# okieraised/rs-face-detection

Hardware: AMD Instinct MI355X
Metric: images/sec + p50 latency, RetinaFace-R50 640x640 b32 (end-to-end detect: preprocess + CNN + decode + NMS; `value` = frames resident in HBM, `value_host_path` = SURVEY 8(d)'s H2D -> ... -> D2H figure) (higher is better)
Workload: dtype bf16; 1 GPU; RetinaFace-ResNet50 640x640 batch=32 bf16 per GPU (BASELINE.json configs[2]); batch_per_gpu=32, global_batch=32, max_det=1024, parallelism=single GPU

## Files before the change

### include/rfd.h

```cpp
#ifndef RFD_H
#define RFD_H

#include <stddef.h>
#include <stdint.h>

#ifdef __cplusplus
extern "C" {
#endif

#define RFD_VERSION 1

#if defined(__GNUC__)
#define RFD_API __attribute__((visibility("default")))
#else
#define RFD_API
#endif

typedef enum rfd_status {
    RFD_OK = 0,
    RFD_ERR_INVALID_ARG = -1,
    RFD_ERR_NO_DEVICE = -2,
    RFD_ERR_HIP = -3,
    RFD_ERR_CAPACITY = -4,
    RFD_ERR_STATE = -5,
// ... 144 lines not shown
    float minimum_face_ratio;
} rfd_selection_config;
RFD_API void rfd_selection_config_default(rfd_selection_config *cfg);
RFD_API int rfd_select_faces(rfd_ctx *ctx, const rfd_dets *dets, const int *img_h, const int *img_w, int n,
                             const rfd_selection_config *cfg, int is_enroll, float *out_box, float *out_kps,
                             int32_t *found);
RFD_API int rfd_detect_select_batch(rfd_ctx *ctx, const rfd_image *imgs, int n, const rfd_selection_config *cfg,
                                    int is_enroll, float *out_box, float *out_kps, int32_t *found);

RFD_API int rfd_host_alloc(size_t bytes, void **ptr);
RFD_API int rfd_host_free(void *ptr);
RFD_API int rfd_submit_batch(rfd_ctx *ctx, const rfd_image *imgs, int n);
RFD_API int rfd_collect_batch(rfd_ctx *ctx, rfd_dets *out, int *n_out);

typedef struct rfd_alignment_config {
    int32_t out_w, out_h;
    float standard_landmarks[10];
    int32_t reserved[4];
} rfd_alignment_config;
RFD_API void rfd_alignment_config_default(rfd_alignment_config *cfg);
RFD_API int rfd_align_faces(rfd_ctx *ctx, const rfd_image *imgs, int n, const float *boxes, const float *kps,
                            const int32_t *found, const rfd_alignment_config *cfg, uint8_t *out_crops,
                            int32_t *status);
RFD_API int rfd_detect_select_align_batch(rfd_ctx *ctx, const rfd_image *imgs, int n,
                                          const rfd_selection_config *sel_cfg, int is_enroll,
                                          const rfd_alignment_config *align_cfg, float *out_box, float *out_kps,
                                          int32_t *found, uint8_t *out_crops, int32_t *status);

#define RFD_MAX_FACE_TENSORS 4
typedef struct rfd_face_tensor_config {
    int32_t out_w, out_h;
    float   mean[3];
    float   scale[3];
    int32_t reserved[4];
} rfd_face_tensor_config;
RFD_API void rfd_face_tensor_config_quality(rfd_face_tensor_config *cfg);
RFD_API void rfd_face_tensor_config_extraction(rfd_face_tensor_config *cfg);
RFD_API int rfd_face_tensors(rfd_ctx *ctx, const uint8_t *crops, int n, int crop_w, int crop_h,
                             const rfd_face_tensor_config *cfgs, int k, float *const *tensors);
RFD_API int rfd_detect_select_align_tensors_batch(rfd_ctx *ctx, const rfd_image *imgs, int n,
                                                  const rfd_selection_config *sel_cfg, int is_enroll,
                                                  const rfd_alignment_config *align_cfg, float *out_box, float *out_kps,
                                                  int32_t *found, uint8_t *out_crops, int32_t *status,
                                                  const rfd_face_tensor_config *cfgs, int k, float *const *tensors);
RFD_API int rfd_align_faces_tensors(rfd_ctx *ctx, const rfd_image *imgs, int n, const float *boxes, const float *kps,
                                    const int32_t *found, const rfd_alignment_config *cfg, uint8_t *out_crops,
                                    int32_t *status, const rfd_face_tensor_config *cfgs, int k, float *const *tensors);
typedef struct rfd_faces {
    float *box;
    float *kps;
    int32_t *found;
    uint8_t *crops;
    int32_t *status;
    float *tensors[RFD_MAX_FACE_TENSORS];
} rfd_faces;
RFD_API int rfd_detect_faces_device(rfd_ctx *ctx, const rfd_image *imgs, int n, const rfd_selection_config *sel_cfg,
                                    int is_enroll, const rfd_alignment_config *align_cfg,
                                    const rfd_face_tensor_config *cfgs, int k, rfd_faces *out, int async);
RFD_API int rfd_quality_decide(rfd_ctx *ctx, const float *logits, int n, int classes, float threshold, float *score,
                               int32_t *klass);
RFD_API int rfd_normalize_embeddings(rfd_ctx *ctx, const float *emb, int n, int dim, float *out);
RFD_API int rfd_quality_decide_device(rfd_ctx *ctx, const float *logits, int n, int classes, float threshold, float *score,
                                      int32_t *klass);
RFD_API int rfd_normalize_embeddings_device(rfd_ctx *ctx, const float *emb, int n, int dim, float *out);

RFD_API int rfd_get_stats(rfd_ctx *ctx, rfd_stats *stats);
RFD_API int rfd_get_config(const rfd_ctx *ctx, rfd_config *cfg);
RFD_API int rfd_set_thresholds(rfd_ctx *ctx, float confidence_threshold, float iou_threshold);
RFD_API int rfd_set_profiling(rfd_ctx *ctx, int enable);
RFD_API int rfd_get_conv_profile(rfd_ctx *ctx, float *ms_conv, double *flops_conv, int *launches);
RFD_API int rfd_get_op_profile(rfd_ctx *ctx, float *ms, int cap);

RFD_API int rfd_debug_tensor_io(rfd_ctx *ctx, int tensor_id, int n, void *host, int write);
RFD_API int rfd_debug_run_ops(rfd_ctx *ctx, int n, int first_op, int last_op);
RFD_API int rfd_debug_run_chain(rfd_ctx *ctx, int n, int first_op, int last_op, int batch_off, int co_running);
RFD_API int rfd_debug_pass_chains(rfd_ctx *ctx, int n, int *sizes, int cap);
RFD_API int rfd_debug_buffer_io(rfd_ctx *ctx, int tensor_id, void *host, size_t bytes, int write, size_t *image_pitch);
RFD_API int rfd_debug_set_conv_tile(rfd_ctx *ctx, int tile);
RFD_API int rfd_debug_op_kernels(rfd_ctx *ctx, int n, int op, int co_running, char *names, int cap);
RFD_API int rfd_debug_op_kernels_static(int backbone, int net_w, int net_h, int n, int op, int co_running, int tile, int schedule,
                                        int cus, char *names, int cap);
RFD_API int rfd_debug_set_concurrency(rfd_ctx *ctx, int multi_stream, int split_min_part, int split_max_parts,
                                      int use_graph);

RFD_API int rfd_debug_poke_nms_flag(rfd_ctx *ctx, int value);
RFD_API int rfd_debug_persistent_kernel(int i, const char **name, size_t *lds_bytes);

#ifdef __cplusplus
}
#endif
#endif
```

### rs-face-detection_amd/csrc/detector.hip

```cpp
#include <dlfcn.h>
#include <stdarg.h>
#include <stdlib.h>

#include <mutex>
#include <vector>

#include "network.h"

namespace rfd {

static thread_local char g_err[512] = "";

void set_error(const char *fmt, ...)
{
    va_list ap;
    va_start(ap, fmt);
    vsnprintf(g_err, sizeof g_err, fmt, ap);
    va_end(ap);
}
const char *get_error() { return g_err; }

static void make_base_anchors(float out[kNumLevels][kA][4])
{
    static const float scales[kNumLevels][kA] = {{32.f, 16.f}, {8.f, 4.f}, {2.f, 1.f}};
// ... 98 lines not shown
    g_rccl = r;
    return RFD_OK;
}

#define RFD_RCCL(expr)                                                                                      \
    do {                                                                                                    \
        const int _r = (expr);                                                                              \
        if (_r != 0) {                                                                                      \
            ::rfd::set_error("%s failed: %s (%s:%d)", #expr, g_rccl.GetErrorString(_r), __FILE__, __LINE__); \
            return RFD_ERR_COMM;                                                                            \
        }                                                                                                   \
    } while (0)

struct DevBuf {
    void *p = nullptr;
    size_t cap = 0;
    int reserve(size_t bytes)
    {
        if (bytes <= cap) return RFD_OK;
        if (p) RFD_HIP(hipFree(p));
        p = nullptr; cap = 0;
        RFD_HIP(hipMalloc(&p, bytes));
        cap = bytes;
        return RFD_OK;
    }
    void release() { if (p) (void)hipFree(p); p = nullptr; cap = 0; }
};

}

using namespace rfd;

struct rfd_ctx {
    rfd_config cfg;
    hipStream_t stream = nullptr;
    hipStream_t own_stream = nullptr;
    hipEvent_t ev[10] = {};
    float base_anchor[kNumLevels][kA][4];
    int fh[kNumLevels], fw[kNumLevels], level_off[kNumLevels], total_anchors = 0;
    Network net;
    bool net_created = false;
    DevBuf staging, imgs, in4, rows, keys, sorted_keys, sorted_boxes, count, det_scale;
    DevBuf nms_kept, nms_state;
    int nms_epoch = 0;
    int nms_ticket_sel = 0;
    bool nms_chunked = true;
    int *h_nms_flag = nullptr;
    DevBuf out_boxes, out_lmk, out_count, out_total, out_gidx;
    DevBuf scratch[12];
    DevBuf sel_dims, sel_out;
    DevBuf align_faces, align_out, align_status;
    DevBuf face_in, face_tensors[kMaxFaceTensors], face_io[2];
    static constexpr int kRing = 4;
    PreImage *pin_imgs[kRing] = {};
    float *pin_scales[kRing] = {};
    hipEvent_t pin_done[kRing] = {};
    int pin_next = 0;
    int *pin_dims[kRing] = {};
    hipEvent_t pin_dims_done[kRing] = {};
    int pin_dims_next = 0;
    struct PipeSlot {
        DevBuf frames, imgs, scale, ob, ol, oc, ot;
        PreImage *pin_imgs = nullptr;
        float *pin_scale = nullptr;
        float *h_ob = nullptr, *h_ol = nullptr;
        int *h_oc = nullptr, *h_ot = nullptr;
        hipEvent_t h2d = nullptr, done = nullptr, post = nullptr;
        int n = 0;
    };
    static constexpr int kPipe = 2;
    static constexpr int kPipeRows = 128;
    PipeSlot pipe[kPipe];
    hipStream_t copy_stream = nullptr, d2h_stream = nullptr;
    int pipe_head = 0, pipe_tail = 0, pipe_inflight = 0;
    DevBuf ov_imgs[2], ov_scale[2];
    hipEvent_t ov_chain_done[2][2] = {}, ov_post_done[2] = {}, ov_desc = nullptr;
    bool ov_post_valid[2] = {false, false};
    int ov_parity = 0;
    int ov_last_n = -1;
    hipEvent_t ov_resync = nullptr;
    Rccl::Comm comm = nullptr;
    int comm_rank = 0, comm_world = 0;
    rfd_stats stats;
    float conv_ms = 0.f;
    double conv_flops = 0.0;
    int conv_launches = 0;

    int ensure_network()
    {
        if (net_created) return RFD_OK;
        RFD_TRY(net.create(cfg.backbone, cfg.image_w, cfg.image_h, cfg.max_batch_size, cfg.precision, cfg.schedule));
        net.d_fail = (int *)nms_state.p + (size_t)cfg.max_batch_size * kNmsChunks * 2;
        net_created = true;
        return RFD_OK;
    }
};

namespace {

int ctx_alloc(rfd_ctx *c)
{
    const size_t B = (size_t)c->cfg.max_batch_size, NA = (size_t)c->total_anchors, MD = (size_t)c->cfg.max_det;
    RFD_TRY(c->imgs.reserve(B * sizeof(PreImage)));
    RFD_TRY(c->rows.reserve(B * NA * kDetRow * sizeof(float)));
    RFD_TRY(c->keys.reserve(B * NA * sizeof(uint64_t)));
    RFD_TRY(c->sorted_keys.reserve(B * NA * sizeof(uint64_t)));
    RFD_TRY(c->sorted_boxes.reserve(B * NA * sizeof(float4)));
    RFD_TRY(c->nms_kept.reserve(B * NA * sizeof(float4)));
    RFD_TRY(c->nms_state.reserve((B * kNmsChunks * 2 + 4) * sizeof(int)));
    RFD_HIP(hipMemset(c->nms_state.p, 0, (B * kNmsChunks * 2 + 4) * sizeof(int)));
    RFD_HIP(hipDeviceSynchronize());
    RFD_TRY(c->count.reserve(B * sizeof(int)));
    RFD_TRY(c->det_scale.reserve(B * sizeof(float)));
    RFD_TRY(c->out_boxes.reserve(B * MD * 5 * sizeof(float)));
    RFD_TRY(c->out_lmk.reserve(B * MD * 10 * sizeof(float)));
    RFD_TRY(c->out_count.reserve(B * sizeof(int)));
    RFD_TRY(c->out_total.reserve(B * sizeof(int)));
    RFD_TRY(c->out_gidx.reserve(B * MD * sizeof(int)));
    return RFD_OK;
}

int check_images(const rfd_ctx *c, const rfd_image *imgs, int n)
{
    RFD_CHECK_ARG(imgs != nullptr, "imgs is null");
    if (n < 1 || n > c->cfg.max_batch_size) {
        set_error("batch of %d frames exceeds max_batch_size %d", n, c->cfg.max_batch_size);
        return RFD_ERR_CAPACITY;
    }
    for (int i = 0; i < n; ++i) {
        RFD_CHECK_ARG(imgs[i].data != nullptr, "frame data is null");
        RFD_CHECK_ARG(imgs[i].height > 0 && imgs[i].width > 0, "frame has a non-positive size");
        RFD_CHECK_ARG(imgs[i].stride >= (ptrdiff_t)imgs[i].width * 3, "frame stride < width*3 (frames must be 3-channel 8-bit)");
    }
    return RFD_OK;
}

int stage_frames(rfd_ctx *c, const rfd_image *imgs, int n, bool frames_on_device, std::vector<float> &scales)
{
    const int slot = c->pin_next;
    c->pin_next = (c->pin_next + 1) % rfd_ctx::kRing;
    RFD_HIP(hipEventSynchronize(c->pin_done[slot]));
    PreImage *pis = c->pin_imgs[slot];
    scales.resize(n);
    size_t total = 0;
    for (int i = 0; i < n; ++i) total += (size_t)imgs[i].height * imgs[i].width * 3;
    if (!frames_on_device) RFD_TRY(c->staging.reserve(total));
    size_t off = 0;
    for (int i = 0; i < n; ++i) {
        letterbox(imgs[i].height, imgs[i].width, c->cfg.image_w, c->cfg.image_h, &pis[i], &scales[i]);
        if (pis[i].new_w <= 0 || pis[i].new_h <= 0) {
            set_error("invalid argument: frame %d (%dx%d) letterboxes to an empty %dx%d image", i, imgs[i].width,
                      imgs[i].height, pis[i].new_w, pis[i].new_h);
            return RFD_ERR_INVALID_ARG;
        }
        if (frames_on_device) {
            pis[i].src = imgs[i].data;
            pis[i].stride = (long long)imgs[i].stride;
        } else {
            uint8_t *dst = (uint8_t *)c->staging.p + off;
            const size_t row = (size_t)imgs[i].width * 3;
            RFD_HIP(hipMemcpy2DAsync(dst, row, imgs[i].data, (size_t)imgs[i].stride, row, imgs[i].height,
                                     hipMemcpyHostToDevice, c->stream));
            pis[i].src = dst;
            pis[i].stride = (long long)row;
            off += row * imgs[i].height;
        }
    }
    memcpy(c->pin_scales[slot], scales.data(), n * sizeof(float));
    RFD_HIP(hipMemcpyAsync(c->imgs.p, pis, n * sizeof(PreImage), hipMemcpyHostToDevice, c->stream));
    RFD_HIP(hipMemcpyAsync(c->det_scale.p, c->pin_scales[slot], n * sizeof(float), hipMemcpyHostToDevice, c->stream));
    RFD_HIP(hipEventRecord(c->pin_done[slot], c->stream));
    return RFD_OK;
}

void fill_decode_params(const rfd_ctx *c, DecodeParams &p)
{
    memset(&p, 0, sizeof p);
    for (int l = 0; l < kNumLevels; ++l) {
        p.fh[l] = c->fh[l]; p.fw[l] = c->fw[l]; p.stride[l] = kStrides[l]; p.level_off[l] = c->level_off[l];
    }
    memcpy(p.base_anchor, c->base_anchor, sizeof p.base_anchor);
    p.total_anchors = c->total_anchors;
    p.net_h = c->cfg.image_h; p.net_w = c->cfg.image_w;
    p.conf_thr = c->cfg.confidence_threshold;
    p.rows = (float *)c->rows.p;
    p.keys = (uint64_t *)c->keys.p;
    p.count = (int *)c->count.p;
}

int post_network(rfd_ctx *c, DecodeParams &dp, bool nchw, int n, float *oboxes, float *olmk, int *ocount,
                 int *ototal, int *ogidx, const float *det_scale = nullptr)
{
    RFD_HIP(hipMemsetAsync(c->count.p, 0, n * sizeof(int), c->stream));
    RFD_TRY(launch_decode(dp, n, nchw, c->stream));
    RFD_HIP(hipEventRecord(c->ev[4], c->stream));
    RFD_TRY(launch_sort((uint64_t *)c->keys.p, (const int *)c->count.p, (const float *)c->rows.p,
                        (uint64_t *)c->sorted_keys.p, (float4 *)c->sorted_boxes.p, c->total_anchors, n, c->stream));
    RFD_HIP(hipEventRecord(c->ev[5], c->stream));
    NmsParams np;
    memset(&np, 0, sizeof np);
    np.sorted_keys = (const uint64_t *)c->sorted_keys.p;
    np.sorted_boxes = (const float4 *)c->sorted_boxes.p;
    np.rows = (const float *)c->rows.p;
    np.count = (const int *)c->count.p;
    np.det_scale = det_scale ? det_scale : (const float *)c->det_scale.p;
    np.presorted_n = -1;
    np.total_anchors = c->total_anchors;
    np.max_det = c->cfg.max_det;
    np.iou_thr = c->cfg.iou_threshold;
    np.out_boxes = oboxes; np.out_lmk = olmk; np.out_count = ocount; np.out_total = ototal; np.out_gidx = ogidx;
    if (c->nms_chunked) {
        np.kept_boxes = (float4 *)c->nms_kept.p;
        np.chunk_state = (int *)c->nms_state.p;
        np.spin_fail = (int *)c->nms_state.p + (size_t)c->cfg.max_batch_size * kNmsChunks * 2;
        np.ticket = (unsigned *)(np.spin_fail + 2);
        np.ticket_sel = c->nms_ticket_sel;
        c->nms_epoch = c->nms_epoch == 0x7fffffff ? 1 : c->nms_epoch + 1;
        np.epoch = c->nms_epoch;
    }
    bool used_chunked = false;
    RFD_TRY(launch_nms(np, n, c->stream, &used_chunked));
    if (used_chunked) c->nms_ticket_sel ^= 1;
    RFD_HIP(hipEventRecord(c->ev[6], c->stream));
    RFD_HIP(hipMemcpyAsync(c->h_nms_flag, (int *)c->nms_state.p + (size_t)c->cfg.max_batch_size * kNmsChunks * 2, sizeof(int), hipMemcpyDeviceToHost, c->stream));
    return RFD_OK;
}

int check_nms_flag(rfd_ctx *c)
{
    if (!c->h_nms_flag || *c->h_nms_flag == 0) return RFD_OK;
    *c->h_nms_flag = 0;
    int *flag = (int *)c->nms_state.p + (size_t)c->cfg.max_batch_size * kNmsChunks * 2;
    RFD_HIP(hipMemsetAsync(flag, 0, sizeof(int), c->stream));
    RFD_HIP(hipStreamSynchronize(c->stream));
    set_error("a device-side bounded wait gave up (chunked NMS: a workgroup waiting for its predecessor chunk; ring convolution: a "
              "wave waiting for a ring slot; split-K convolution: an arrival counter left dirty by an earlier fault); the detections of the batches since the last synchronisation are invalid "
              "(re-submit them; RFD_NMS_CHUNKED=0 selects the one-workgroup-per-image NMS kernel, RFD_CONV_RING=0 the barrier-per-step convolutions)");
    return RFD_ERR_HIP;
}

int finish_stats(rfd_ctx *c, int n, bool have_pre, bool have_net)
{
    float ms;
    memset(&c->stats, 0, sizeof c->stats);
    auto el = [&](int a, int b) { return hipEventElapsedTime(&ms, c->ev[a], c->ev[b]) == hipSuccess ? ms : 0.f; };
    if (have_pre) { c->stats.ms_h2d = el(0, 1); c->stats.ms_preprocess = el(1, 2); }
    if (have_net) c->stats.ms_network = el(2, 3);
    c->stats.ms_decode = el(3, 4);
    c->stats.ms_sort = el(4, 5);
    c->stats.ms_nms = el(5, 6);
    c->stats.ms_d2h = el(6, 7);
    c->stats.ms_total = el(have_pre ? 0 : (have_net ? 2 : 3), 7);
    std::vector<int> cnt(n), tot(n);
    RFD_HIP(hipMemcpy(cnt.data(), c->count.p, n * sizeof(int), hipMemcpyDeviceToHost));
    for (int i = 0; i < n; ++i) c->stats.candidates += cnt[i];
    if (c->net_created && c->net.profiling) {
        RFD_TRY(c->net.collect_profile());
        c->conv_ms = 0.f; c->conv_flops = 0.0; c->conv_launches = 0;
        for (size_t i = 0; i < c->net.g.ops.size(); ++i)
            if (c->net.g.ops[i].kind == OP_CONV || c->net.g.ops[i].kind == OP_B2B) {
                c->conv_ms += c->net.op_ms[i];
                c->conv_flops += 2.0 * c->net.g.layer_macs((int)i) * n;
                ++c->conv_launches;
            }
    }
    return RFD_OK;
}

int detect_overlapped(rfd_ctx *c, const rfd_image *imgs, int n, rfd_dets *out, hipEvent_t frames_ready = nullptr)
{
    Network &net = c->net;
    RFD_TRY(net.ensure_alt_heads());
    const size_t B = (size_t)c->cfg.max_batch_size;
    if (!c->ov_desc) {
        RFD_HIP(hipEventCreateWithFlags(&c->ov_desc, hipEventDisableTiming));
        RFD_HIP(hipEventCreateWithFlags(&c->ov_resync, hipEventDisableTiming));
        for (int a = 0; a < 2; ++a) {
            RFD_HIP(hipEventCreateWithFlags(&c->ov_post_done[a], hipEventDisableTiming));
            for (int b = 0; b < 2; ++b) RFD_HIP(hipEventCreateWithFlags(&c->ov_chain_done[a][b], hipEventDisableTiming));
            RFD_TRY(c->ov_imgs[a].reserve(B * sizeof(PreImage)));
            RFD_TRY(c->ov_scale[a].reserve(B * sizeof(float)));
        }
    }
    const int par = (c->ov_parity ^= 1);
    const int slot = c->pin_next;
    c->pin_next = (c->pin_next + 1) % rfd_ctx::kRing;
    RFD_HIP(hipEventSynchronize(c->pin_done[slot]));
    PreImage *pis = c->pin_imgs[slot];
    for (int i = 0; i < n; ++i) {
        letterbox(imgs[i].height, imgs[i].width, c->cfg.image_w, c->cfg.image_h, &pis[i], &c->pin_scales[slot][i]);
        if (pis[i].new_w <= 0 || pis[i].new_h <= 0) {
            set_error("invalid argument: frame %d (%dx%d) letterboxes to an empty image", i, imgs[i].width, imgs[i].height);
            return RFD_ERR_INVALID_ARG;
        }
        pis[i].src = imgs[i].data;
        pis[i].stride = (long long)imgs[i].stride;
    }
    hipStream_t st[2] = {net.part_stream[0], net.part_stream[1]};
    if (c->ov_last_n != n) {
        RFD_HIP(hipEventRecord(c->ov_resync, c->stream));
        for (int p = 0; p < 2; ++p) RFD_HIP(hipStreamWaitEvent(st[p], c->ov_resync, 0));
    }
    c->ov_last_n = n;
    if (frames_ready)
        for (int p = 0; p < 2; ++p) RFD_HIP(hipStreamWaitEvent(st[p], frames_ready, 0));
    if (c->ov_post_valid[par])
        for (int p = 0; p < 2; ++p) RFD_HIP(hipStreamWaitEvent(st[p], c->ov_post_done[par], 0));
    RFD_HIP(hipMemcpyAsync(c->ov_imgs[par].p, pis, n * sizeof(PreImage), hipMemcpyHostToDevice, st[0]));
    RFD_HIP(hipMemcpyAsync(c->ov_scale[par].p, c->pin_scales[slot], n * sizeof(float), hipMemcpyHostToDevice, st[0]));
    RFD_HIP(hipEventRecord(c->pin_done[slot], st[0]));
    RFD_HIP(hipEventRecord(c->ov_desc, st[0]));
    RFD_HIP(hipStreamWaitEvent(st[1], c->ov_desc, 0));
    net.head_parity = par;
    net.co_running = 1;
    int chain[Network::kMaxParts];
    if (net.pass_chains(n, chain) != 2) { set_error("overlapped calls run as two chains"); return RFD_ERR_STATE; }
    const int B0 = chain[0];
    const size_t in_px = (size_t)c->cfg.image_h * c->cfg.image_w * 4;
    int status = RFD_OK;
    for (int p = 0; p < 2 && status == RFD_OK; ++p) {
        const int off = p ? B0 : 0, Bp = chain[p];
        PreParams pp;
        memset(&pp, 0, sizeof pp);
        pp.imgs = (const PreImage *)c->ov_imgs[par].p + off;
        pp.net_h = c->cfg.image_h; pp.net_w = c->cfg.image_w;
        pp.out_nhwc4 = (bf16_t *)net.tensor_ptr(net.g.input) + (size_t)off * in_px;
        status = launch_preprocess(pp, Bp, st[p]);
        if (status == RFD_OK) status = net.run(Bp, st[p], 0, -1, off, p);
        if (status == RFD_OK && hipEventRecord(c->ov_chain_done[par][p], st[p]) != hipSuccess) status = RFD_ERR_HIP;
    }
    net.co_running = 0;
    if (status != RFD_OK) { net.head_parity = 0; c->ov_last_n = -1; return status; }
    for (int p = 0; p < 2; ++p) RFD_HIP(hipStreamWaitEvent(c->stream, c->ov_chain_done[par][p], 0));
    DecodeParams dp;
    fill_decode_params(c, dp);
    for (int l = 0; l < kNumLevels; ++l) dp.cls[l] = (const float *)net.tensor_ptr(net.g.heads[l]);
    net.head_parity = 0;
    RFD_TRY(post_network(c, dp, false, n, out->boxes, out->landmarks, out->count, out->total, nullptr,
                         (const float *)c->ov_scale[par].p));
    RFD_HIP(hipEventRecord(c->ov_post_done[par], c->stream));
    c->ov_post_valid[par] = true;
    return RFD_OK;
}

int detect_impl(rfd_ctx *c, const rfd_image *imgs, int n, rfd_dets *out, bool on_device, int async, bool frames_on_device)
{
    RFD_CHECK_ARG(c != nullptr, "ctx is null");
    RFD_CHECK_ARG(out && out->boxes && out->landmarks && out->count, "output buffers are null");
    RFD_TRY(check_images(c, imgs, n));
    RFD_TRY(c->ensure_network());
    if (!c->net.weights_ready) { set_error("network weights are not initialised"); return RFD_ERR_STATE; }
    if (async == 2 && on_device && frames_on_device && !c->net.profiling && c->net.multi_stream && c->net.num_parts(n) == 2) {
        RFD_HIP(hipSetDevice(c->cfg.device_id));
        return detect_overlapped(c, imgs, n, out);
    }
    RFD_HIP(hipSetDevice(c->cfg.device_id));
    c->ov_last_n = -1;
    std::vector<float> scales;
    RFD_HIP(hipEventRecord(c->ev[0], c->stream));
    RFD_TRY(stage_frames(c, imgs, n, frames_on_device, scales));
    RFD_HIP(hipEventRecord(c->ev[1], c->stream));
    PreParams pp;
    memset(&pp, 0, sizeof pp);
    pp.imgs = (const PreImage *)c->imgs.p;
    pp.net_h = c->cfg.image_h; pp.net_w = c->cfg.image_w;
    pp.out_nhwc4 = (bf16_t *)c->net.tensor_ptr(c->net.g.input);
    RFD_TRY(launch_preprocess(pp, n, c->stream));
    RFD_HIP(hipEventRecord(c->ev[2], c->stream));
    RFD_TRY(c->net.run_graphed(n, c->stream));
    RFD_HIP(hipEventRecord(c->ev[3], c->stream));
    DecodeParams dp;
    fill_decode_params(c, dp);
    for (int l = 0; l < kNumLevels; ++l) dp.cls[l] = (const float *)c->net.tensor_ptr(c->net.g.heads[l]);
    float *ob = on_device ? out->boxes : (float *)c->out_boxes.p;
    float *ol = on_device ? out->landmarks : (float *)c->out_lmk.p;
    int *oc = on_device ? out->count : (int *)c->out_count.p;
    int *ot = on_device ? out->total : (int *)c->out_total.p;
    RFD_TRY(post_network(c, dp, false, n, ob, ol, oc, ot, nullptr));
    if (!on_device) {
        const size_t MD = (size_t)c->cfg.max_det;
        RFD_HIP(hipMemcpyAsync(out->boxes, ob, n * MD * 5 * sizeof(float), hipMemcpyDeviceToHost, c->stream));
        RFD_HIP(hipMemcpyAsync(out->landmarks, ol, n * MD * 10 * sizeof(float), hipMemcpyDeviceToHost, c->stream));
        RFD_HIP(hipMemcpyAsync(out->count, oc, n * sizeof(int), hipMemcpyDeviceToHost, c->stream));
        if (out->total) RFD_HIP(hipMemcpyAsync(out->total, ot, n * sizeof(int), hipMemcpyDeviceToHost, c->stream));
    }
    RFD_HIP(hipEventRecord(c->ev[7], c->stream));
    if (async && on_device) return RFD_OK;
    RFD_HIP(hipStreamSynchronize(c->stream));
    RFD_TRY(check_nms_flag(c));
    RFD_TRY(finish_stats(c, n, true, true));
    if (!on_device)
        for (int i = 0; i < n; ++i) c->stats.detections += out->total ? out->total[i] : out->count[i];
    return RFD_OK;
}

std::mutex g_nms_mu;
rfd_ctx *g_nms_ctx[16] = {};

}

extern "C" {

void rfd_config_default(rfd_config *cfg)
{
    if (!cfg) return;
    memset(cfg, 0, sizeof *cfg);
    cfg->image_w = 640;
    cfg->image_h = 640;
    cfg->max_batch_size = 1;
    cfg->confidence_threshold = 0.7f;
    cfg->iou_threshold = 0.45f;
    cfg->device_id = 0;
    cfg->max_det = 1024;
    cfg->max_src_w = 3840;
    cfg->max_src_h = 2160;
    cfg->backbone = RFD_BACKBONE_R50;
}

int rfd_version(void) { return RFD_VERSION; }
const char *rfd_last_error(void) { return get_error(); }

int rfd_create(const rfd_config *cfg, rfd_ctx **out)
{
    RFD_CHECK_ARG(cfg && out, "cfg/out is null");
    *out = nullptr;
    RFD_CHECK_ARG(cfg->image_w > 0 && cfg->image_h > 0 && cfg->image_w % 32 == 0 && cfg->image_h % 32 == 0,
                  "image_size must be positive multiples of 32");
    RFD_CHECK_ARG(cfg->max_batch_size >= 1, "max_batch_size < 1");
    RFD_CHECK_ARG(cfg->max_det >= 1, "max_det < 1");
    RFD_CHECK_ARG(cfg->precision == RFD_PRECISION_BF16 || cfg->precision == RFD_PRECISION_F32, "precision must be RFD_PRECISION_BF16 or RFD_PRECISION_F32");
    RFD_CHECK_ARG(cfg->precision == RFD_PRECISION_BF16 || cfg->backbone == RFD_BACKBONE_R50, "the f32 parity mode exists for RetinaFace-R50 only");
    RFD_CHECK_ARG(cfg->schedule == RFD_SCHEDULE_THROUGHPUT || cfg->schedule == RFD_SCHEDULE_LATENCY, "schedule must be RFD_SCHEDULE_THROUGHPUT or RFD_SCHEDULE_LATENCY");
    RFD_CHECK_ARG(cfg->schedule == RFD_SCHEDULE_THROUGHPUT || cfg->precision == RFD_PRECISION_BF16, "the latency schedule exists for the bf16 path only (not the f32 parity mode)");
    int ndev = 0;
    if (hipGetDeviceCount(&ndev) != hipSuccess || ndev <= 0) {
        set_error("no HIP device is available: librfd_hip has no CPU fallback");
        return RFD_ERR_NO_DEVICE;
    }
    if (cfg->device_id < 0 || cfg->device_id >= ndev) {
        set_error("device_id %d out of range (%d devices)", cfg->device_id, ndev);
        return RFD_ERR_NO_DEVICE;
    }
    if (hipSetDevice(cfg->device_id) != hipSuccess) {
        set_error("hipSetDevice(%d) failed", cfg->device_id);
        return RFD_ERR_NO_DEVICE;
    }
    rfd_ctx *c = new rfd_ctx();
    c->cfg = *cfg;
    if (const char *e = getenv("RFD_NMS_CHUNKED")) c->nms_chunked = atoi(e) != 0;
    make_base_anchors(c->base_anchor);
    int off = 0;
    for (int l = 0; l < kNumLevels; ++l) {
// ... 170 lines not shown
    return RFD_OK;
}
int rfd_graph_op(const rfd_graph *gg, int idx, rfd_op_desc *d)
{
    RFD_CHECK_ARG(gg && d, "null argument");
    const Graph *g = reinterpret_cast<const Graph *>(gg);
    RFD_CHECK_ARG(idx >= 0 && idx < (int)g->ops.size(), "op index out of range");
    const Op &o = g->ops[idx];
    memset(d, 0, sizeof *d);
    d->kind = o.kind; d->layer = o.layer; d->in = o.in; d->out = o.out; d->out2 = o.out2; d->outf = o.outf;
    d->res = o.res; d->relu = o.relu; d->res_up2 = o.res_up2; d->res_post = o.res_post;
    d->head_softmax = o.head_softmax; d->y_coff = o.y_coff;
    d->in2 = o.in2; d->layer2 = o.layer2; d->in_affine = o.in_affine;
    d->layer_n2 = o.layer_n2; d->x_coff = o.x_coff; d->y_split = o.y_split; d->y_split_add = o.y_split_add;
    d->n_valid = o.n_valid; d->layer_b = o.layer_b; d->out_b = o.out_b; d->branch = o.branch;
    d->macs = g->layer_macs(idx);
    return RFD_OK;
}
int rfd_graph_tensor(const rfd_graph *gg, int idx, rfd_tensor_desc *d)
{
    RFD_CHECK_ARG(gg && d, "null argument");
    const Graph *g = reinterpret_cast<const Graph *>(gg);
    RFD_CHECK_ARG(idx >= 0 && idx < (int)g->tensors.size(), "tensor index out of range");
    const TensorDesc &t = g->tensors[idx];
    memset(d, 0, sizeof *d);
    d->channels = t.C; d->channels_logical = t.C_logical; d->height = t.H; d->width = t.W; d->is_f32 = t.is_f32;
    d->buffer = t.buffer;
    d->is_input = idx == g->input;
    for (int l = 0; l < 3; ++l)
        if (g->heads[l] == idx) d->head_level = l + 1;
    return RFD_OK;
}
double rfd_graph_macs(const rfd_graph *gg)
{
    return gg ? reinterpret_cast<const Graph *>(gg)->macs_per_image() : 0.0;
}
double rfd_graph_workspace_bytes(const rfd_graph *gg)
{
    if (!gg) return 0.0;
    double s = 0;
    for (size_t b : reinterpret_cast<const Graph *>(gg)->buffer_bytes_per_image) s += (double)b;
    return s;
}

int rfd_debug_tensor_io(rfd_ctx *c, int tensor_id, int n, void *host, int write)
{
    RFD_CHECK_ARG(c && host, "null argument");
    RFD_HIP(hipSetDevice(c->cfg.device_id));
    RFD_TRY(c->ensure_network());
    RFD_CHECK_ARG(tensor_id >= 0 && tensor_id < (int)c->net.g.tensors.size(), "tensor id out of range");
    RFD_CHECK_ARG(n >= 1 && n <= c->cfg.max_batch_size, "batch out of range");
    const size_t bytes = c->net.g.tensors[tensor_id].bytes_per_image() * (size_t)n;
    c->ov_last_n = -1;
    if (c->net.precision != 0 && !c->net.g.tensors[tensor_id].is_f32 && tensor_id != c->net.g.input) {
        set_error("f32 parity mode: intermediate tensors are f32, not the bf16 layout this hook transfers");
        return RFD_ERR_STATE;
    }
    if (write) RFD_HIP(hipMemcpyAsync(c->net.tensor_ptr(tensor_id), host, bytes, hipMemcpyHostToDevice, c->stream));
    else RFD_HIP(hipMemcpyAsync(host, c->net.tensor_ptr(tensor_id), bytes, hipMemcpyDeviceToHost, c->stream));
    RFD_HIP(hipStreamSynchronize(c->stream));
    return RFD_OK;
}
int rfd_debug_set_conv_tile(rfd_ctx *c, int tile)
{
    RFD_CHECK_ARG(c && tile >= 0 && tile <= 31, "bad argument");
    RFD_TRY(c->ensure_network());
    c->net.force_tile = tile;
    return RFD_OK;
}
int rfd_debug_set_concurrency(rfd_ctx *c, int multi_stream, int split_min_part, int split_max_parts, int use_graph)
{
    RFD_CHECK_ARG(c, "ctx is null");
    RFD_TRY(c->ensure_network());
    RFD_HIP(hipStreamSynchronize(c->stream));
    c->net.multi_stream = multi_stream != 0;
    c->net.split_min_part = split_min_part;
    c->net.split_max_parts = split_max_parts;
    c->net.tuned = false;
    c->net.use_graph = use_graph != 0;
    for (hipGraphExec_t &ge : c->net.graph_exec)
        if (ge) { (void)hipGraphExecDestroy(ge); ge = nullptr; }
    return RFD_OK;
}
int rfd_debug_poke_nms_flag(rfd_ctx *c, int value)
{
    RFD_CHECK_ARG(c, "ctx is null");
    RFD_HIP(hipSetDevice(c->cfg.device_id));
    int *flag = (int *)c->nms_state.p + (size_t)c->cfg.max_batch_size * kNmsChunks * 2;
    RFD_HIP(hipMemcpyAsync(flag, &value, sizeof(int), hipMemcpyHostToDevice, c->stream));
    RFD_HIP(hipStreamSynchronize(c->stream));
    return RFD_OK;
}
int rfd_debug_persistent_kernel(int i, const char **name, size_t *lds_bytes) { return rfd::persistent_kernel_table(i, name, lds_bytes); }
int rfd_debug_run_ops(rfd_ctx *c, int n, int first_op, int last_op)
{
    RFD_CHECK_ARG(c, "ctx is null");
    RFD_HIP(hipSetDevice(c->cfg.device_id));
    RFD_TRY(c->ensure_network());
    c->ov_last_n = -1;
    RFD_TRY(c->net.run(n, c->stream, first_op, last_op));
    RFD_HIP(hipMemcpyAsync(c->h_nms_flag, c->net.d_fail, sizeof(int), hipMemcpyDeviceToHost, c->stream));
    RFD_HIP(hipStreamSynchronize(c->stream));
    if (c->net.profiling) RFD_TRY(c->net.collect_profile());
    return check_nms_flag(c);
}

int rfd_debug_run_chain(rfd_ctx *c, int n, int first_op, int last_op, int batch_off, int co_running)
{
    RFD_CHECK_ARG(c, "ctx is null");
    RFD_HIP(hipSetDevice(c->cfg.device_id));
    RFD_TRY(c->ensure_network());
    RFD_CHECK_ARG(n >= 1 && batch_off >= 0 && batch_off + n <= c->cfg.max_batch_size, "chain [batch_off, batch_off + n) out of range");
    c->ov_last_n = -1;
    const int saved = c->net.co_running;
    c->net.co_running = co_running != 0;
    const int st = c->net.run(n, c->stream, first_op, last_op, batch_off, 0);
    c->net.co_running = saved;
    RFD_TRY(st);
    RFD_HIP(hipMemcpyAsync(c->h_nms_flag, c->net.d_fail, sizeof(int), hipMemcpyDeviceToHost, c->stream));
    RFD_HIP(hipStreamSynchronize(c->stream));
    if (c->net.profiling) RFD_TRY(c->net.collect_profile());
    return check_nms_flag(c);
}
int rfd_debug_pass_chains(rfd_ctx *c, int n, int *sizes, int cap)
{
    RFD_CHECK_ARG(c && sizes, "null argument");
    RFD_TRY(c->ensure_network());
    RFD_CHECK_ARG(n >= 1 && n <= c->cfg.max_batch_size, "batch out of range");
    int chain[Network::kMaxParts];
    const int P = c->net.pass_chains(n, chain);
    RFD_CHECK_ARG(cap >= P, "sizes holds fewer entries than the pass has chains");
    for (int p = 0; p < P; ++p) sizes[p] = chain[p];
    return P;
}
int rfd_debug_buffer_io(rfd_ctx *c, int tensor_id, void *host, size_t bytes, int write, size_t *image_pitch)
{
    RFD_CHECK_ARG(c, "ctx is null");
    RFD_HIP(hipSetDevice(c->cfg.device_id));
    RFD_TRY(c->ensure_network());
    RFD_CHECK_ARG(tensor_id >= 0 && tensor_id < (int)c->net.g.tensors.size(), "tensor id out of range");
    if (c->net.precision != 0) { set_error("f32 parity mode keeps its own workspace"); return RFD_ERR_STATE; }
    const size_t pitch = c->net.g.buffer_bytes_per_image[c->net.g.tensors[tensor_id].buffer];
    if (image_pitch) *image_pitch = pitch;
    if (!host) return RFD_OK;
    RFD_CHECK_ARG(bytes == pitch * (size_t)c->cfg.max_batch_size, "bytes is not the size of the buffer (max_batch_size * image pitch)");
    c->ov_last_n = -1;
    if (write) RFD_HIP(hipMemcpyAsync(c->net.tensor_ptr(tensor_id), host, bytes, hipMemcpyHostToDevice, c->stream));
    else RFD_HIP(hipMemcpyAsync(host, c->net.tensor_ptr(tensor_id), bytes, hipMemcpyDeviceToHost, c->stream));
    RFD_HIP(hipStreamSynchronize(c->stream));
    return RFD_OK;
}

int rfd_debug_op_kernels(rfd_ctx *c, int n, int op, int co_running, char *names, int cap)
{
    RFD_CHECK_ARG(c && names && cap > 0, "null argument");
    RFD_HIP(hipSetDevice(c->cfg.device_id));
    RFD_TRY(c->ensure_network());
    RFD_CHECK_ARG(n >= 1 && n <= c->cfg.max_batch_size && op >= 0 && op < (int)c->net.g.ops.size(), "batch or op out of range");
    if (c->net.precision != 0) { set_error("kernel-choice introspection covers the bf16 path"); return RFD_ERR_STATE; }
    if (!c->net.weights_ready) { set_error("network weights are not initialised (rfd_init_synthetic_weights / rfd_set_layer_weights)"); return RFD_ERR_STATE; }
    const int saved = c->net.co_running;
    c->net.co_running = co_running != 0;
    std::string out;
    const int st = c->net.op_kernel_names(n, op, device_cus(), &out);
    c->net.co_running = saved;
    RFD_TRY(st);
    snprintf(names, (size_t)cap, "%s", out.c_str());
    return RFD_OK;
}

int rfd_debug_op_kernels_static(int backbone, int net_w, int net_h, int n, int op, int co_running, int tile, int schedule, int cus, char *names, int cap)
{
    RFD_CHECK_ARG(names && cap > 0 && n >= 1 && cus >= 1 && tile >= 0 && tile <= 31, "bad argument");
    Network net;
    RFD_TRY(net.g.build(backbone, net_w, net_h));
    RFD_CHECK_ARG(op >= 0 && op < (int)net.g.ops.size(), "op out of range");
    net.max_batch = n;
    net.schedule = schedule;
    net.force_tile = tile;
    net.co_running = co_running != 0;
    if (schedule == RFD_SCHEDULE_LATENCY) (void)net.plan_splitk();
    char *const base = reinterpret_cast<char *>((uintptr_t)1 << 32);
    net.d_w = reinterpret_cast<bf16_t *>(base);
    net.d_b = reinterpret_cast<float *>(base);
    net.d_zero = reinterpret_cast<bf16_t *>(base);
    net.d_buffers.assign(net.g.buffer_bytes_per_image.size(), base);
    for (int b = 0; b < 3; ++b) net.d_sk_ws[b] = reinterpret_cast<float *>(base);
    net.d_sk_cnt = reinterpret_cast<unsigned *>(base);
    std::string out;
    RFD_TRY(net.op_kernel_names(n, op, cus, &out));
    snprintf(names, (size_t)cap, "%s", out.c_str());
    return RFD_OK;
}

int rfd_init_synthetic_weights(rfd_ctx *c, uint64_t seed)
{
    RFD_CHECK_ARG(c, "ctx is null");
    RFD_HIP(hipSetDevice(c->cfg.device_id));
    RFD_TRY(c->ensure_network());
    return c->net.init_synthetic(seed, c->stream);
}
int rfd_num_layers(const rfd_ctx *c)
{
    if (!c || !c->net_created) return 0;
    return (int)c->net.g.layers.size();
// ... 198 lines not shown
}
int rfd_host_free(void *ptr)
{
    if (ptr) RFD_HIP(hipHostFree(ptr));
    return RFD_OK;
}

int rfd_submit_batch(rfd_ctx *c, const rfd_image *imgs, int n)
{
    RFD_CHECK_ARG(c != nullptr, "ctx is null");
    RFD_TRY(check_images(c, imgs, n));
    if (c->pipe_inflight >= rfd_ctx::kPipe) {
        set_error("%d batches are already in flight: call rfd_collect_batch first", c->pipe_inflight);
        return RFD_ERR_STATE;
    }
    RFD_HIP(hipSetDevice(c->cfg.device_id));
    RFD_TRY(c->ensure_network());
    const size_t B = (size_t)c->cfg.max_batch_size, MD = (size_t)c->cfg.max_det;
    rfd_ctx::PipeSlot &ps = c->pipe[c->pipe_head];
    if (!c->copy_stream) RFD_HIP(hipStreamCreateWithFlags(&c->copy_stream, hipStreamNonBlocking));
    if (!ps.done) {
        RFD_HIP(hipEventCreateWithFlags(&ps.h2d, hipEventDisableTiming));
        RFD_HIP(hipEventCreateWithFlags(&ps.done, hipEventDisableTiming));
        RFD_HIP(hipHostMalloc((void **)&ps.pin_imgs, B * sizeof(PreImage), hipHostMallocDefault));
        RFD_HIP(hipHostMalloc((void **)&ps.pin_scale, B * sizeof(float), hipHostMallocDefault));
        RFD_HIP(hipHostMalloc((void **)&ps.h_ob, B * MD * 5 * sizeof(float), hipHostMallocDefault));
        RFD_HIP(hipHostMalloc((void **)&ps.h_ol, B * MD * 10 * sizeof(float), hipHostMallocDefault));
        RFD_HIP(hipHostMalloc((void **)&ps.h_oc, B * sizeof(int), hipHostMallocDefault));
        RFD_HIP(hipHostMalloc((void **)&ps.h_ot, B * sizeof(int), hipHostMallocDefault));
        RFD_TRY(ps.imgs.reserve(B * sizeof(PreImage)));
        RFD_TRY(ps.scale.reserve(B * sizeof(float)));
        RFD_TRY(ps.ob.reserve(B * MD * 5 * sizeof(float)));
        RFD_TRY(ps.ol.reserve(B * MD * 10 * sizeof(float)));
        RFD_TRY(ps.oc.reserve(B * sizeof(int)));
        RFD_TRY(ps.ot.reserve(B * sizeof(int)));
    }
    size_t total = 0;
    for (int i = 0; i < n; ++i) total += (size_t)imgs[i].height * imgs[i].width * 3;
    if (total > ps.frames.cap) {
        RFD_TRY(ps.frames.reserve(total + total / 4));
    }
    size_t off = 0;
    for (int i = 0; i < n; ++i) {
        letterbox(imgs[i].height, imgs[i].width, c->cfg.image_w, c->cfg.image_h, &ps.pin_imgs[i], &ps.pin_scale[i]);
        if (ps.pin_imgs[i].new_w <= 0 || ps.pin_imgs[i].new_h <= 0) {
            set_error("invalid argument: frame %d (%dx%d) letterboxes to an empty image", i, imgs[i].width, imgs[i].height);
            return RFD_ERR_INVALID_ARG;
        }
        ps.pin_imgs[i].src = (uint8_t *)ps.frames.p + off;
        ps.pin_imgs[i].stride = (long long)imgs[i].width * 3;
        off += (size_t)imgs[i].width * 3 * imgs[i].height;
    }
    for (int i = 0; i < n;) {
        size_t bytes = (size_t)imgs[i].width * 3 * imgs[i].height;
        int j = i + 1;
        if (imgs[i].stride == (ptrdiff_t)imgs[i].width * 3) {
            while (j < n && imgs[j].stride == (ptrdiff_t)imgs[j].width * 3 && imgs[j].data == imgs[i].data + bytes) {
                bytes += (size_t)imgs[j].width * 3 * imgs[j].height;
                ++j;
            }
            RFD_HIP(hipMemcpyAsync((void *)ps.pin_imgs[i].src, imgs[i].data, bytes, hipMemcpyHostToDevice, c->copy_stream));
        } else {
            const size_t row = (size_t)imgs[i].width * 3;
            RFD_HIP(hipMemcpy2DAsync((void *)ps.pin_imgs[i].src, row, imgs[i].data, (size_t)imgs[i].stride, row, imgs[i].height,
                                     hipMemcpyHostToDevice, c->copy_stream));
        }
        i = j;
    }
    RFD_HIP(hipMemcpyAsync(ps.imgs.p, ps.pin_imgs, n * sizeof(PreImage), hipMemcpyHostToDevice, c->copy_stream));
    RFD_HIP(hipMemcpyAsync(ps.scale.p, ps.pin_scale, n * sizeof(float), hipMemcpyHostToDevice, c->copy_stream));
    RFD_HIP(hipEventRecord(ps.h2d, c->copy_stream));
    if (!c->net.profiling && c->net.multi_stream && c->net.num_parts(n) == 2 && c->net.weights_ready) {
        std::vector<rfd_image> dev(n);
        for (int i = 0; i < n; ++i) {
            dev[i].data = (const uint8_t *)ps.pin_imgs[i].src; dev[i].height = imgs[i].height; dev[i].width = imgs[i].width;
            dev[i].stride = (ptrdiff_t)imgs[i].width * 3;
        }
        rfd_dets dd;
        dd.boxes = (float *)ps.ob.p; dd.landmarks = (float *)ps.ol.p; dd.count = (int *)ps.oc.p; dd.total = (int *)ps.ot.p;
        RFD_TRY(detect_overlapped(c, dev.data(), n, &dd, ps.h2d));
    } else {
        c->ov_last_n = -1;
        RFD_HIP(hipStreamWaitEvent(c->stream, ps.h2d, 0));
        PreParams pp;
        memset(&pp, 0, sizeof pp);
        pp.imgs = (const PreImage *)ps.imgs.p;
        pp.net_h = c->cfg.image_h; pp.net_w = c->cfg.image_w;
        pp.out_nhwc4 = (bf16_t *)c->net.tensor_ptr(c->net.g.input);
        RFD_TRY(launch_preprocess(pp, n, c->stream));
        RFD_TRY(c->net.run_graphed(n, c->stream));
        DecodeParams dp;
        fill_decode_params(c, dp);
        for (int l = 0; l < kNumLevels; ++l) dp.cls[l] = (const float *)c->net.tensor_ptr(c->net.g.heads[l]);
        RFD_TRY(post_network(c, dp, false, n, (float *)ps.ob.p, (float *)ps.ol.p, (int *)ps.oc.p, (int *)ps.ot.p, nullptr,
                             (const float *)ps.scale.p));
    }
    if (!c->d2h_stream) RFD_HIP(hipStreamCreateWithFlags(&c->d2h_stream, hipStreamNonBlocking));
    if (!ps.post) RFD_HIP(hipEventCreateWithFlags(&ps.post, hipEventDisableTiming));
    RFD_HIP(hipEventRecord(ps.post, c->stream));
    RFD_HIP(hipStreamWaitEvent(c->d2h_stream, ps.post, 0));
    const size_t R = std::min<size_t>(MD, rfd_ctx::kPipeRows);
    RFD_HIP(hipMemcpy2DAsync(ps.h_ob, MD * 5 * sizeof(float), ps.ob.p, MD * 5 * sizeof(float), R * 5 * sizeof(float), n, hipMemcpyDeviceToHost, c->d2h_stream));
    RFD_HIP(hipMemcpy2DAsync(ps.h_ol, MD * 10 * sizeof(float), ps.ol.p, MD * 10 * sizeof(float), R * 10 * sizeof(float), n, hipMemcpyDeviceToHost, c->d2h_stream));
    RFD_HIP(hipMemcpyAsync(ps.h_oc, ps.oc.p, n * sizeof(int), hipMemcpyDeviceToHost, c->d2h_stream));
    RFD_HIP(hipMemcpyAsync(ps.h_ot, ps.ot.p, n * sizeof(int), hipMemcpyDeviceToHost, c->d2h_stream));
    RFD_HIP(hipEventRecord(ps.done, c->d2h_stream));
    ps.n = n;
    c->pipe_head = (c->pipe_head + 1) % rfd_ctx::kPipe;
    ++c->pipe_inflight;
    return RFD_OK;
}

int rfd_collect_batch(rfd_ctx *c, rfd_dets *out, int *n_out)
{
    RFD_CHECK_ARG(c && out && out->boxes && out->landmarks && out->count, "null argument");
    if (c->pipe_inflight <= 0) { set_error("no batch in flight"); return RFD_ERR_STATE; }
    rfd_ctx::PipeSlot &ps = c->pipe[c->pipe_tail];
    RFD_HIP(hipEventSynchronize(ps.done));
    if (*c->h_nms_flag) {
        c->pipe_tail = (c->pipe_tail + 1) % rfd_ctx::kPipe;
        --c->pipe_inflight;
        return check_nms_flag(c);
    }
    const size_t MD = (size_t)c->cfg.max_det;
    bool more = false;
    for (int i = 0; i < ps.n; ++i)
        if ((size_t)ps.h_oc[i] > (size_t)rfd_ctx::kPipeRows) {
            const size_t R = rfd_ctx::kPipeRows, k = (size_t)ps.h_oc[i];
            RFD_HIP(hipMemcpyAsync(ps.h_ob + ((size_t)i * MD + R) * 5, (const float *)ps.ob.p + ((size_t)i * MD + R) * 5, (k - R) * 5 * sizeof(float), hipMemcpyDeviceToHost, c->d2h_stream));
            RFD_HIP(hipMemcpyAsync(ps.h_ol + ((size_t)i * MD + R) * 10, (const float *)ps.ol.p + ((size_t)i * MD + R) * 10, (k - R) * 10 * sizeof(float), hipMemcpyDeviceToHost, c->d2h_stream));
            more = true;
        }
    if (more) RFD_HIP(hipStreamSynchronize(c->d2h_stream));
    for (int i = 0; i < ps.n; ++i) {
        const int k = ps.h_oc[i];
        memcpy(out->boxes + (size_t)i * MD * 5, ps.h_ob + (size_t)i * MD * 5, (size_t)k * 5 * sizeof(float));
        memcpy(out->landmarks + (size_t)i * MD * 10, ps.h_ol + (size_t)i * MD * 10, (size_t)k * 10 * sizeof(float));
        out->count[i] = k;
        if (out->total) out->total[i] = ps.h_ot[i];
    }
    if (n_out) *n_out = ps.n;
    c->pipe_tail = (c->pipe_tail + 1) % rfd_ctx::kPipe;
    --c->pipe_inflight;
    return RFD_OK;
}

int rfd_preprocess(rfd_ctx *c, const rfd_image *imgs, int n, uint8_t *det_img, float *tensor, float *det_scale)
{
    RFD_CHECK_ARG(c != nullptr, "ctx is null");
    RFD_TRY(check_images(c, imgs, n));
    RFD_HIP(hipSetDevice(c->cfg.device_id));
    std::vector<float> scales;
    RFD_TRY(stage_frames(c, imgs, n, false, scales));
    const size_t npix = (size_t)n * c->cfg.image_h * c->cfg.image_w;
    PreParams pp;
    memset(&pp, 0, sizeof pp);
    pp.imgs = (const PreImage *)c->imgs.p;
    pp.net_h = c->cfg.image_h; pp.net_w = c->cfg.image_w;
    if (det_img) { RFD_TRY(c->scratch[0].reserve(npix * 3)); pp.out_det_img = (uint8_t *)c->scratch[0].p; }
    if (tensor) { RFD_TRY(c->scratch[1].reserve(npix * 3 * sizeof(float))); pp.out_tensor = (float *)c->scratch[1].p; }
    RFD_TRY(launch_preprocess(pp, n, c->stream));
    if (det_img) RFD_HIP(hipMemcpyAsync(det_img, pp.out_det_img, npix * 3, hipMemcpyDeviceToHost, c->stream));
    if (tensor) RFD_HIP(hipMemcpyAsync(tensor, pp.out_tensor, npix * 3 * sizeof(float), hipMemcpyDeviceToHost, c->stream));
    RFD_HIP(hipStreamSynchronize(c->stream));
    if (det_scale) memcpy(det_scale, scales.data(), n * sizeof(float));
    return RFD_OK;
}

int rfd_forward(rfd_ctx *c, const float *tensor, int n, float *const heads[9])
{
    RFD_CHECK_ARG(c && tensor && heads, "null argument");
    for (int i = 0; i < 9; ++i) RFD_CHECK_ARG(heads[i] != nullptr, "head pointer is null");
    if (n < 1 || n > c->cfg.max_batch_size) { set_error("batch %d exceeds max_batch_size %d", n, c->cfg.max_batch_size); return RFD_ERR_CAPACITY; }
// ... 512 lines not shown
```

### rs-face-detection_amd/csrc/kernels.h

```cpp
#pragma once
#include "rfd_common.h"

namespace rfd {

struct PreImage {
    const uint8_t *src;
    long long stride;
    int h, w;
    int new_w, new_h;
    int area_fast;
    int pad;
    double scale_x, scale_y;
};

struct PreParams {
    const PreImage *imgs;
    int net_h, net_w;
    bf16_t *out_nhwc4;
    uint8_t *out_det_img;
    float *out_tensor;
};
int launch_preprocess(const PreParams &p, int n, hipStream_t s);
int launch_tensor_to_nhwc4(const float *tensor, bf16_t *out, int n, int H, int W, hipStream_t s);

// ... 198 lines not shown
    X(K_PW_PAIR_2_1_RAW_4, "pw_pair_kernel<2, 1, false, 4, 0, false>")                                \
    X(K_PW_PAIR_4_2_RAW, "pw_pair_kernel<4, 2, false, 0, 0, false>")                                  \
    X(K_PW_PAIR_2_2_ACT, "pw_pair_kernel<2, 2, true, 0, 0, false>")                                   \
    X(K_PW_PAIR_1_1_ACT_0_2, "pw_pair_kernel<1, 1, true, 0, 2, false>")                               \
    X(K_PW_PAIR_1_1_RAW_1_2_HALF, "pw_pair_kernel<1, 1, false, 1, 2, true>")                          \
    X(K_PW_PAIR_1_1_RAW_0_2_HALF, "pw_pair_kernel<1, 1, false, 0, 2, true>")                          \
    X(K_PW_GEMM, "pw_gemm_kernel<false, false>")                                                      \
    X(K_PW_GEMM_WIDE, "pw_gemm_kernel<false, true>")                                                  \
    X(K_PW_GEMM_AFF, "pw_gemm_kernel<true, false>")                                                   \
    X(K_PW_GEMM_AFF_WIDE, "pw_gemm_kernel<true, true>")                                               \
    X(K_PW_WIDE, "pw_wide_kernel")                                                                    \
    X(K_RING, "conv_ring_kernel<false>")                                                              \
    X(K_RING_KX3, "conv_ring_kernel<true>")                                                           \
    X(K_SPLITK_64_64_2_2, "conv_splitk_kernel<64, 64, 2, 2>")
enum ConvKernel : int {
    K_NONE = 0,
#define RFD_ID(id, name) id,
    RFD_CONV_KERNELS(RFD_ID)
#undef RFD_ID
};
const char *conv_kernel_name(ConvKernel k);

struct ConvStep {
    ConvKernel kernel;
    ConvParams p;
};
struct ConvPlan {
    int steps;
    ConvStep step[2];
};
static inline bool bank_behind(const bf16_t *w, const bf16_t *w1) { return (uintptr_t)w1 > (uintptr_t)w && (uintptr_t)w1 - (uintptr_t)w < (1u << 30); }
int choose_conv(const ConvParams &p, bool w1_behind_w, ConvPlan *plan);
int launch_conv(const ConvParams &p, hipStream_t s);

constexpr int kSplitKMaxSegments = 8;
struct SplitKPlan {
    int S, bm, bn;
    int tiles;
    size_t ws_bytes;
};
int conv_splitk_segments(int nk);
bool conv_splitk_plan(int K, int Cout, int HoWo, int B, SplitKPlan *pl);
bool conv_splitk_wants(const ConvParams &p, SplitKPlan *pl);
int launch_conv_splitk(const ConvParams &p, hipStream_t s);
bool conv_ring_supports(const ConvParams &p, bool *kx3);
int launch_conv_ring(const ConvParams &p, hipStream_t s);
int device_cus();
int persistent_kernel_table(int i, const char **name, size_t *lds_bytes);
struct ConvF32Params {
    const float *x, *w, *x2;
    const float *bias, *bias2;
    const float *res;
    const float *in_scale, *in_shift, *scale2, *shift2;
    float *y, *y2, *yf;
    int B, H, W, Cin, Cout, KH, KW, stride, pad, Ho, Wo;
    int H2, W2, Cin2, stride2;
    int ldw;
    int ldy, y_coff, ldx, x_coff, y_split, y_split_add, n_valid;
    int relu, res_up2, res_post, head_softmax;
};
int launch_conv_f32(const ConvF32Params &p, hipStream_t s);
int launch_conv0_f32(const bf16_t *x4, const float *w, const float *bias, float *y, int B, int H, int W, hipStream_t s);
int launch_maxpool_f32(const float *x, float *y, const float *scale, const float *shift, int B, int H, int W, int C, hipStream_t s);

struct B2BParams {
    const bf16_t *x, *x2;
    const bf16_t *w3;
    const float *bias3, *bias3b;
    const bf16_t *res;
    const float *scale, *shift;
    bf16_t *raw;
    const bf16_t *w1;
    const float *bias1;
    bf16_t *t1;
    int B, H, W, Cin, Cin2;
    int force_tile;
};
void choose_b2b_s1(const B2BParams &p, bool w1_behind_w3, ConvStep *st);
int launch_conv_b2b_s1(const B2BParams &p, hipStream_t s);
constexpr int kStemPH = 4, kStemPW = 16;
ConvKernel choose_stem(int B, int H, int W, bool conv1_offered, int force_tile, int cus);
int launch_stem(const bf16_t *x4, const bf16_t *w, const float *bias, const float *scale, const float *shift,
                bf16_t *y, int B, int H, int W, hipStream_t s, int force_tile = 0, const bf16_t *w1 = nullptr,
                const float *bias1 = nullptr, bf16_t *t1 = nullptr, bool *fused = nullptr);
int launch_first3x3(const bf16_t *x4, const bf16_t *w, const float *bias, bf16_t *y, int B, int H, int W, int Cd,
                    hipStream_t s);
int launch_dwconv3x3(const bf16_t *x, const bf16_t *w, const float *bias, bf16_t *y, int B, int H, int W, int C,
                     int stride, hipStream_t s);
int launch_heads_to_nchw(const float *h32, float *cls, float *bbox, float *lmk, int B, int fh,
                         int fw, hipStream_t s);

}
```

### rs-face-detection_amd/csrc/kernels_conv.hip

```cpp
#include "conv_device.h"

namespace rfd {


template <int N> __device__ __forceinline__ void wait_vmcnt()
{
    static_assert(N == 0, "counted vmcnt waits are not used: drain");
    asm volatile("s_waitcnt vmcnt(0)" ::: "memory");
}

#ifdef RFD_CLOCK_STAMPS
__device__ unsigned long long g_clock_stamps[16][2];
struct ClockStamp {
    unsigned long long t0, r0;
    int cls;
    __device__ ClockStamp(int c) : cls(c) { t0 = __builtin_amdgcn_s_memtime(); r0 = __builtin_amdgcn_s_memrealtime(); }
    __device__ ~ClockStamp()
    {
        const unsigned long long dt = __builtin_amdgcn_s_memtime() - t0, dr = __builtin_amdgcn_s_memrealtime() - r0;
        if (threadIdx.x == 0) {
            atomicAdd(&g_clock_stamps[cls][0], dt);
            atomicAdd(&g_clock_stamps[cls][1], dr);
        }
    }
};
#define RFD_CLOCK(cls) ClockStamp clock_stamp__(cls)
extern "C" __attribute__((visibility("default"))) int rfd_debug_clock_stamps(unsigned long long *out, int reset)
{
    static unsigned long long host[32];
    if (hipMemcpyFromSymbol(host, HIP_SYMBOL(g_clock_stamps), sizeof host) != hipSuccess) return -1;
    for (int i = 0; i < 32; ++i) out[i] = host[i];
    if (reset) { memset(host, 0, sizeof host); if (hipMemcpyToSymbol(HIP_SYMBOL(g_clock_stamps), host, sizeof host) != hipSuccess) return -1; }
    return 0;
}
#else
#define RFD_CLOCK(cls) do { } while (0)
#endif
template <int BM, int BN, int WAVES_M, int WAVES_N, int NSX, bool CHUNK_MAJOR = false>
__global__ void __launch_bounds__(WAVES_M *WAVES_N * 64) conv_igemm_kernel(const ConvParams p)
{
    RFD_CLOCK(0);
    constexpr int NT = WAVES_M * WAVES_N * 64, NW = WAVES_M * WAVES_N;
    constexpr int WM = BM / WAVES_M, WN = BN / WAVES_N;
    constexpr int TM = WM / 16, TN = WN / 16;
    constexpr int XP = BM / 8 / NW, WP = (BN / 8 + NW - 1) / NW;
    static_assert((BM / 8) % NW == 0, "X tile pieces must divide over the waves");

    extern __shared__ __attribute__((aligned(16))) unsigned char smem[];
    bf16_t *Xs = reinterpret_cast<bf16_t *>(smem);

    const int tid = threadIdx.x, lane = tid & 63;
    const int wave = __builtin_amdgcn_readfirstlane(tid >> 6);
    const int wm = wave % WAVES_M, wn = wave / WAVES_M;
    const int HoWo = p.Ho * p.Wo;
    const int M = p.B * HoWo;
    const int K1 = p.KH * p.KW * p.Cin;
    const int K = K1 + p.Cin2;
    const int nk1 = K1 >> 6, nk = K >> 6;
    bf16_t *Ws = Xs + (nk > 1 ? NSX : 1) * BM * 64;
    const int tiles_n = p.Cout / BN;
    const int lid = xcd_remap(blockIdx.x, gridDim.x);
    const int m0 = (lid / tiles_n) * BM, n0 = (lid % tiles_n) * BN;

    const int lr = lane >> 3, chunk = (lane & 7) ^ lr;
    const __amdgpu_buffer_rsrc_t rx = __builtin_amdgcn_make_buffer_rsrc(
        const_cast<bf16_t *>(p.x), 0, (uint32_t)((size_t)p.B * p.H * p.W * p.ldx * 2), 0x00020000);
    const __amdgpu_buffer_rsrc_t rw = __builtin_amdgcn_make_buffer_rsrc(
        const_cast<bf16_t *>(p.w), 0, (uint32_t)((size_t)p.Cout * K * 2), 0x00020000);
    const __amdgpu_buffer_rsrc_t rx2 = __builtin_amdgcn_make_buffer_rsrc(
        const_cast<bf16_t *>(p.Cin2 ? p.x2 : p.x), 0,
        (uint32_t)(p.Cin2 ? (size_t)p.B * p.H2 * p.W2 * p.Cin2 * 2 : 0), 0x00020000);
    uint32_t xoff[XP], xoff2[XP];
    int hi0[XP], wi0[XP];
#pragma unroll
    for (int q = 0; q < XP; ++q) {
        const int m = m0 + (wave + NW * q) * 8 + lr;
        xoff2[q] = kOob;
        if (m < M) {
            const int b = m / HoWo, rem = m - b * HoWo;
            const int ho = rem / p.Wo, wo = rem - ho * p.Wo;
            hi0[q] = ho * p.stride - p.pad;
            wi0[q] = wo * p.stride - p.pad;
            xoff[q] = (uint32_t)(((((long long)b * p.H + hi0[q]) * p.W + wi0[q]) * p.ldx + p.x_coff + chunk * 8) * 2);
// ... 2419 lines not shown
    float bv[2][8];
#pragma unroll
    for (int h = 0; h < 2; ++h) {
        const float4 b0 = *reinterpret_cast<const float4 *>(bias + h * 32 + fq * 8);
        const float4 b1 = *reinterpret_cast<const float4 *>(bias + h * 32 + fq * 8 + 4);
        bv[h][0] = b0.x; bv[h][1] = b0.y; bv[h][2] = b0.z; bv[h][3] = b0.w;
        bv[h][4] = b1.x; bv[h][5] = b1.y; bv[h][6] = b1.z; bv[h][7] = b1.w;
    }
    constexpr int NPIX = kStemCR * kStemCC, NT16 = (NPIX + 15) / 16;
    for (int t = wave; t < NT16; t += 4) {
        const int idx = min(t * 16 + frow, NPIX - 1);
        const int cr = idx / kStemCC, cc = idx - cr * kStemCC;
        const uint2 *ip = in_tile + (2 * cr) * kStemIP + 2 * cc + 2 * fq;
        f32x4 acc[4];
#pragma unroll
        for (int i = 0; i < 4; ++i) acc[i] = f32x4{0.f, 0.f, 0.f, 0.f};
#pragma unroll
        for (int k = 0; k < 7; ++k) {
            const bf16x8 bf = *reinterpret_cast<const bf16x8 *>(ip + k * kStemIP);
#pragma unroll
            for (int i = 0; i < 4; ++i)
                acc[i] = __builtin_amdgcn_mfma_f32_16x16x32_bf16(af[i][k], bf, acc[i], 0, 0, 0);
        }
        if (t * 16 + frow < NPIX) {
            const int gr = cr0 + cr, gc = cc0 + cc;
            const uint32_t inside = ((unsigned)gr < (unsigned)Ho && (unsigned)gc < (unsigned)Wo) ? 0xffffffffu : 0u;
#pragma unroll
            for (int h = 0; h < 2; ++h) {
                float o[8];
#pragma unroll
                for (int k = 0; k < 4; ++k) {
                    o[k] = fmaxf(acc[2 * h][k] + bv[h][k], 0.f);
                    o[4 + k] = fmaxf(acc[2 * h + 1][k] + bv[h][4 + k], 0.f);
                }
                const uint2 lo = pack_bf16x4(o[0], o[1], o[2], o[3]), hi = pack_bf16x4(o[4], o[5], o[6], o[7]);
                *reinterpret_cast<uint4 *>(conv_tile + idx * kStemCP + h * 32 + fq * 8) =
                    make_uint4(lo.x & inside, lo.y & inside, hi.x & inside, hi.y & inside);
            }
        }
    }
    __syncthreads();

    static_assert(kStemPH * kStemPW * 8 % 256 == 0, "the pooling pass runs whole rounds of the workgroup (a scalar trip count)");
    for (int round = 0; round < kStemPH * kStemPW * 8 / 256; ++round) {
        const int item = tid + round * 256;
        const int c8 = item & 7, pp = item >> 3;
        const int pr = pp / kStemPW, pc = pp - pr * kStemPW;
        const bool live = ph0 + pr < Hp && pw0 + pc < Wp;
        typedef short i16x2 __attribute__((ext_vector_type(2)));
        i16x2 mi[4] = {i16x2{0, 0}, i16x2{0, 0}, i16x2{0, 0}, i16x2{0, 0}};
#pragma unroll
        for (int dy = 0; dy < 3; ++dy)
#pragma unroll
            for (int dx = 0; dx < 3; ++dx) {
                const uint4 v = *reinterpret_cast<const uint4 *>(conv_tile + ((2 * pr + dy) * kStemCC + 2 * pc + dx) * kStemCP + c8 * 8);
                const uint32_t u[4] = {v.x, v.y, v.z, v.w};
#pragma unroll
                for (int k = 0; k < 4; ++k) mi[k] = __builtin_elementwise_max(mi[k], __builtin_bit_cast(i16x2, u[k]));
            }
        asm volatile("" : "+v"(mi[0]), "+v"(mi[1]), "+v"(mi[2]), "+v"(mi[3]));
        float mx[8];
#pragma unroll
        for (int k = 0; k < 4; ++k) {
            const uint32_t u = __builtin_bit_cast(uint32_t, mi[k]);
            mx[2 * k] = bf16_bits_to_f32(u & 0xffffu);
            mx[2 * k + 1] = bf16_bits_to_f32(u >> 16);
        }
        const float4 s0 = *reinterpret_cast<const float4 *>(scale + c8 * 8), s1 = *reinterpret_cast<const float4 *>(scale + c8 * 8 + 4);
        const float4 t0 = *reinterpret_cast<const float4 *>(shift + c8 * 8), t1 = *reinterpret_cast<const float4 *>(shift + c8 * 8 + 4);
        const uint2 lo = pack_bf16x4(fmaxf(mx[0] * s0.x + t0.x, 0.f), fmaxf(mx[1] * s0.y + t0.y, 0.f),
                                     fmaxf(mx[2] * s0.z + t0.z, 0.f), fmaxf(mx[3] * s0.w + t0.w, 0.f));
        const uint2 hi = pack_bf16x4(fmaxf(mx[4] * s1.x + t1.x, 0.f), fmaxf(mx[5] * s1.y + t1.y, 0.f),
                                     fmaxf(mx[6] * s1.z + t1.z, 0.f), fmaxf(mx[7] * s1.w + t1.w, 0.f));
        if (live) *reinterpret_cast<uint4 *>(y + (((size_t)b * Hp + ph0 + pr) * Wp + pw0 + pc) * 64 + c8 * 8) = make_uint4(lo.x, lo.y, hi.x, hi.y);
    }
}

template <bool FUSE1>
__global__ void __launch_bounds__(256) stem_persistent_kernel(const bf16_t *__restrict__ x4, const bf16_t *__restrict__ w,
                                                              const float *__restrict__ bias, const float *__restrict__ scale,
                                                              const float *__restrict__ shift, bf16_t *__restrict__ y, int H,
                                                              int W, int tiles_w, int tiles_h, int ntiles, int per,
                                                              const bf16_t *__restrict__ w1, const float *__restrict__ bias1,
                                                              bf16_t *__restrict__ t1)
{
    RFD_CLOCK(12);
    __shared__ __attribute__((aligned(16))) uint2 in_tile[kStemIR * kStemIP];
    __shared__ __attribute__((aligned(16))) bf16_t conv_tile[kStemCR * kStemCC * kStemCP];
    __shared__ __attribute__((aligned(16))) bf16_t w1_tile[FUSE1 ? 64 * 64 : 8];
    const int tid = threadIdx.x, lane = tid & 63, frow = lane & 15, fq = lane >> 4;
    const int wave = __builtin_amdgcn_readfirstlane(tid >> 6);
    const int Ho = H >> 1, Wo = W >> 1, Hp = Ho >> 1, Wp = Wo >> 1;
    const int t_begin = (int)blockIdx.x * per, t_end = min(ntiles, t_begin + per);
    if (t_begin >= t_end) return;
    constexpr int NR = (kStemIR * kStemIP + 255) / 256;
    auto load_patch = [&](int t, uint2 (&pre)[NR]) {
        const int tw_ = t % tiles_w, th_ = (t / tiles_w) % tiles_h, b_ = t / (tiles_w * tiles_h);
        const int ir0_ = 2 * (2 * th_ * kStemPH - 1) - 3, ic0_ = 2 * (2 * tw_ * kStemPW - 1) - 3;
        const uint2 *src_ = reinterpret_cast<const uint2 *>(x4) + (size_t)b_ * H * W;
#pragma unroll
        for (int round = 0; round < NR; ++round) {
            const int i = tid + round * 256;
            const int r = i / kStemIP, c = i - r * kStemIP;
            const int gr = ir0_ + r, gc = ic0_ + c;
            const bool ok = c < kStemIC && (unsigned)gr < (unsigned)H && (unsigned)gc < (unsigned)W;
            const uint32_t keep = ok ? 0xffffffffu : 0u;
            const uint2 v = src_[ok ? (size_t)gr * W + gc : (size_t)0];
            pre[round] = make_uint2(v.x & keep, v.y & keep);
        }
    };
    auto store_patch = [&](const uint2 (&pre)[NR]) {
#pragma unroll
        for (int round = 0; round < NR; ++round) {
            const int i = tid + round * 256;
            if (i < kStemIR * kStemIP) in_tile[i] = pre[round];
        }
    };

    bf16x8 af[4][7];
#pragma unroll
    for (int i = 0; i < 4; ++i) {
        const int chn = (i >> 1) * 32 + (frow >> 2) * 8 + (i & 1) * 4 + (frow & 3);
#pragma unroll
        for (int k = 0; k < 7; ++k)
            af[i][k] = *reinterpret_cast<const bf16x8 *>(w + ((size_t)chn * 7 + k) * 32 + fq * 8);
    }
    uint2 pre[NR];
    load_patch(t_begin, pre);
    store_patch(pre);
    if (FUSE1) {
#pragma unroll
        for (int round = 0; round < 2; ++round) {
            const int idx = tid + round * 256, rho = idx >> 3, c = idx & 7, i = rho >> 4, r = rho & 15;
            const int chn = (i >> 1) * 32 + (r >> 2) * 8 + (i & 1) * 4 + (r & 3);
            *reinterpret_cast<uint4 *>(w1_tile + rho * 64 + ((c ^ (rho & 7)) << 3)) = *reinterpret_cast<const uint4 *>(w1 + chn * 64 + c * 8);
        }
    }
    __syncthreads();

    float bv[2][8];
#pragma unroll
    for (int h = 0; h < 2; ++h) {
        const float4 b0 = *reinterpret_cast<const float4 *>(bias + h * 32 + fq * 8);
        const float4 b1 = *reinterpret_cast<const float4 *>(bias + h * 32 + fq * 8 + 4);
        bv[h][0] = b0.x; bv[h][1] = b0.y; bv[h][2] = b0.z; bv[h][3] = b0.w;
        bv[h][4] = b1.x; bv[h][5] = b1.y; bv[h][6] = b1.z; bv[h][7] = b1.w;
    }
    constexpr int NPIX = kStemCR * kStemCC, NT16 = (NPIX + 15) / 16;
    for (int tile = t_begin; tile < t_end; ++tile) {
        const int tw = tile % tiles_w, th = (tile / tiles_w) % tiles_h, b = tile / (tiles_w * tiles_h);
        const int ph0 = th * kStemPH, pw0 = tw * kStemPW;
        const int cr0 = 2 * ph0 - 1, cc0 = 2 * pw0 - 1;
        const bool more = tile + 1 < t_end;
        if (more) load_patch(tile + 1, pre);
    for (int t = wave; t < NT16; t += 4) {
        const int idx = min(t * 16 + frow, NPIX - 1);
        const int cr = idx / kStemCC, cc = idx - cr * kStemCC;
        const uint2 *ip = in_tile + (2 * cr) * kStemIP + 2 * cc + 2 * fq;
        f32x4 acc[4];
#pragma unroll
        for (int i = 0; i < 4; ++i) acc[i] = f32x4{0.f, 0.f, 0.f, 0.f};
#pragma unroll
        for (int k = 0; k < 7; ++k) {
            const bf16x8 bf = *reinterpret_cast<const bf16x8 *>(ip + k * kStemIP);
#pragma unroll
            for (int i = 0; i < 4; ++i)
                acc[i] = __builtin_amdgcn_mfma_f32_16x16x32_bf16(af[i][k], bf, acc[i], 0, 0, 0);
        }
        if (t * 16 + frow < NPIX) {
            const int gr = cr0 + cr, gc = cc0 + cc;
            const uint32_t inside = ((unsigned)gr < (unsigned)Ho && (unsigned)gc < (unsigned)Wo) ? 0xffffffffu : 0u;
#pragma unroll
            for (int h = 0; h < 2; ++h) {
                float o[8];
#pragma unroll
                for (int k = 0; k < 4; ++k) {
                    o[k] = fmaxf(acc[2 * h][k] + bv[h][k], 0.f);
                    o[4 + k] = fmaxf(acc[2 * h + 1][k] + bv[h][4 + k], 0.f);
                }
                const uint2 lo = pack_bf16x4(o[0], o[1], o[2], o[3]), hi = pack_bf16x4(o[4], o[5], o[6], o[7]);
                *reinterpret_cast<uint4 *>(conv_tile + idx * kStemCP + h * 32 + fq * 8) =
                    make_uint4(lo.x & inside, lo.y & inside, hi.x & inside, hi.y & inside);
            }
        }
    }
        __syncthreads();
        if (more) store_patch(pre);
    static_assert(kStemPH * kStemPW * 8 % 256 == 0, "the pooling pass runs whole rounds of the workgroup (a scalar trip count)");
    static_assert(!FUSE1 || (kStemPW == 16 && kStemPH == 4), "fused conv1: a wave owns one pooled row of 16 pixels");
    uint4 yq[2];
    for (int round = 0; round < kStemPH * kStemPW * 8 / 256; ++round) {
        const int item = tid + round * 256;
        const int c8 = FUSE1 ? round * 4 + fq : item & 7, pp = FUSE1 ? wave * 16 + frow : item >> 3;
        const int pr = pp / kStemPW, pc = pp - pr * kStemPW;
        const bool live = ph0 + pr < Hp && pw0 + pc < Wp;
        typedef short i16x2 __attribute__((ext_vector_type(2)));
        i16x2 mi[4] = {i16x2{0, 0}, i16x2{0, 0}, i16x2{0, 0}, i16x2{0, 0}};
#pragma unroll
        for (int dy = 0; dy < 3; ++dy)
#pragma unroll
            for (int dx = 0; dx < 3; ++dx) {
                const uint4 v = *reinterpret_cast<const uint4 *>(conv_tile + ((2 * pr + dy) * kStemCC + 2 * pc + dx) * kStemCP + c8 * 8);
                const uint32_t u[4] = {v.x, v.y, v.z, v.w};
#pragma unroll
                for (int k = 0; k < 4; ++k) mi[k] = __builtin_elementwise_max(mi[k], __builtin_bit_cast(i16x2, u[k]));
            }
        asm volatile("" : "+v"(mi[0]), "+v"(mi[1]), "+v"(mi[2]), "+v"(mi[3]));
        float mx[8];
#pragma unroll
        for (int k = 0; k < 4; ++k) {
            const uint32_t u = __builtin_bit_cast(uint32_t, mi[k]);
            mx[2 * k] = bf16_bits_to_f32(u & 0xffffu);
            mx[2 * k + 1] = bf16_bits_to_f32(u >> 16);
        }
        const float4 s0 = *reinterpret_cast<const float4 *>(scale + c8 * 8), s1 = *reinterpret_cast<const float4 *>(scale + c8 * 8 + 4);
        const float4 t0 = *reinterpret_cast<const float4 *>(shift + c8 * 8), t1 = *reinterpret_cast<const float4 *>(shift + c8 * 8 + 4);
        const uint2 lo = pack_bf16x4(fmaxf(mx[0] * s0.x + t0.x, 0.f), fmaxf(mx[1] * s0.y + t0.y, 0.f),
                                     fmaxf(mx[2] * s0.z + t0.z, 0.f), fmaxf(mx[3] * s0.w + t0.w, 0.f));
        const uint2 hi = pack_bf16x4(fmaxf(mx[4] * s1.x + t1.x, 0.f), fmaxf(mx[5] * s1.y + t1.y, 0.f),
                                     fmaxf(mx[6] * s1.z + t1.z, 0.f), fmaxf(mx[7] * s1.w + t1.w, 0.f));
        if (live) *reinterpret_cast<uint4 *>(y + (((size_t)b * Hp + ph0 + pr) * Wp + pw0 + pc) * 64 + c8 * 8) = make_uint4(lo.x, lo.y, hi.x, hi.y);
        if (FUSE1) yq[round & 1] = make_uint4(lo.x, lo.y, hi.x, hi.y);
    }
    if (FUSE1) {
        f32x4 a1[4];
#pragma unroll
        for (int i = 0; i < 4; ++i) a1[i] = f32x4{0.f, 0.f, 0.f, 0.f};
#pragma unroll
        for (int kk = 0; kk < 2; ++kk) {
            const bf16x8 bq = __builtin_bit_cast(bf16x8, yq[kk]);
#pragma unroll
            for (int i = 0; i < 4; ++i) {
                const int rho = i * 16 + frow;
                const bf16x8 aw = *reinterpret_cast<const bf16x8 *>(w1_tile + rho * 64 + (((kk * 4 + fq) ^ (rho & 7)) << 3));
                a1[i] = __builtin_amdgcn_mfma_f32_16x16x32_bf16(aw, bq, a1[i], 0, 0, 0);
            }
        }
        const bool live1 = ph0 + wave < Hp && pw0 + frow < Wp;
#pragma unroll
        for (int h = 0; h < 2; ++h) {
            const float4 c0 = *reinterpret_cast<const float4 *>(bias1 + h * 32 + fq * 8), c1 = *reinterpret_cast<const float4 *>(bias1 + h * 32 + fq * 8 + 4);
            const float b1v[8] = {c0.x, c0.y, c0.z, c0.w, c1.x, c1.y, c1.z, c1.w};
            float o[8];
#pragma unroll
            for (int k = 0; k < 4; ++k) {
                o[k] = fmaxf(a1[2 * h][k] + b1v[k], 0.f);
                o[4 + k] = fmaxf(a1[2 * h + 1][k] + b1v[4 + k], 0.f);
            }
            const uint2 lo = pack_bf16x4(o[0], o[1], o[2], o[3]), hi = pack_bf16x4(o[4], o[5], o[6], o[7]);
            if (live1) *reinterpret_cast<uint4 *>(t1 + (((size_t)b * Hp + ph0 + wave) * Wp + pw0 + frow) * 64 + h * 32 + fq * 8) = make_uint4(lo.x, lo.y, hi.x, hi.y);
        }
    }
        __syncthreads();
    }
}


int launch_stem(const bf16_t *x4, const bf16_t *w, const float *bias, const float *scale, const float *shift,
                bf16_t *y, int B, int H, int W, hipStream_t s, int force_tile, const bf16_t *w1, const float *bias1, bf16_t *t1, bool *fused)
{
    if (fused) *fused = false;
    if ((H | W) & 3) {
        set_error("stem: input %dx%d must be a multiple of 4", H, W);
        return RFD_ERR_INVALID_ARG;
    }
    const int Hp = H / 4, Wp = W / 4;
    const int tiles_h = ceil_div(Hp, kStemPH), tiles_w = ceil_div(Wp, kStemPW);
    const int ntiles = B * tiles_h * tiles_w;
    const int slots = 2 * device_cus();
    const int per = ceil_div(ntiles, slots), grid = ceil_div(ntiles, per);
    switch (choose_stem(B, H, W, w1 && t1 && fused, force_tile, device_cus())) {
    case K_STEM_PERSISTENT_CONV1:
        *fused = true;
        hipLaunchKernelGGL(stem_persistent_kernel<true>, dim3((unsigned)grid), dim3(256), 0, s, x4, w, bias, scale, shift, y, H, W, tiles_w, tiles_h, ntiles, per, w1, bias1, t1);
        break;
    case K_STEM_PERSISTENT:
        hipLaunchKernelGGL(stem_persistent_kernel<false>, dim3((unsigned)grid), dim3(256), 0, s, x4, w, bias, scale, shift, y, H, W, tiles_w, tiles_h, ntiles, per, nullptr, nullptr, nullptr);
        break;
    default:
        hipLaunchKernelGGL(stem_kernel, dim3((unsigned)ntiles), dim3(256), 0, s, x4, w, bias, scale, shift, y,
                           H, W, tiles_w, tiles_h);
    }
    RFD_HIP(hipGetLastError());
    return RFD_OK;
}

__global__ void __launch_bounds__(256) first3x3_kernel(const bf16_t *__restrict__ x4, const uint32_t *__restrict__ w2,
                                                       const float *__restrict__ bias, bf16_t *__restrict__ y, int B,
                                                       int H, int W, int Ho, int Wo, int Cd)
{
    const long long i = (long long)blockIdx.x * 256 + threadIdx.x;
    if (i >= (long long)B * Ho * Wo) return;
    const int wo = (int)(i % Wo);
    const int ho = (int)((i / Wo) % Ho);
    const int b = (int)(i / ((long long)Wo * Ho));
    float acc[8];
#pragma unroll
    for (int c = 0; c < 8; ++c) acc[c] = bias[c];
#pragma unroll
    for (int ky = 0; ky < 3; ++ky) {
        const int hi = 2 * ho - 1 + ky;
        if ((unsigned)hi >= (unsigned)H) continue;
#pragma unroll
        for (int kx = 0; kx < 3; ++kx) {
            const int wi = 2 * wo - 1 + kx;
            if ((unsigned)wi >= (unsigned)W) continue;
            const uint2 p = reinterpret_cast<const uint2 *>(x4)[((long long)b * H + hi) * W + wi];
            const float r = bf16_bits_to_f32(p.x & 0xffffu), g = bf16_bits_to_f32(p.x >> 16), bl = bf16_bits_to_f32(p.y & 0xffffu);
#pragma unroll
            for (int c = 0; c < 8; ++c) {
                const uint32_t d0 = w2[c * 18 + (ky * 3 + kx) * 2], d1 = w2[c * 18 + (ky * 3 + kx) * 2 + 1];
                acc[c] += r * bf16_bits_to_f32(d0 & 0xffffu) + g * bf16_bits_to_f32(d0 >> 16) + bl * bf16_bits_to_f32(d1 & 0xffffu);
            }
        }
    }
    uint4 *dst = reinterpret_cast<uint4 *>(y + i * Cd);
    const uint2 lo = pack_bf16x4(fmaxf(acc[0], 0.f), fmaxf(acc[1], 0.f), fmaxf(acc[2], 0.f), fmaxf(acc[3], 0.f));
    const uint2 hi2 = pack_bf16x4(fmaxf(acc[4], 0.f), fmaxf(acc[5], 0.f), fmaxf(acc[6], 0.f), fmaxf(acc[7], 0.f));
    dst[0] = make_uint4(lo.x, lo.y, hi2.x, hi2.y);
    for (int k = 1; k < Cd / 8; ++k) dst[k] = make_uint4(0, 0, 0, 0);
}

int launch_first3x3(const bf16_t *x4, const bf16_t *w, const float *bias, bf16_t *y, int B, int H, int W, int Cd,
                    hipStream_t s)
{
    const int Ho = (H + 2 - 3) / 2 + 1, Wo = (W + 2 - 3) / 2 + 1;
    const long long total = (long long)B * Ho * Wo;
    hipLaunchKernelGGL(first3x3_kernel, dim3((unsigned)((total + 255) / 256)), dim3(256), 0, s, x4,
                       reinterpret_cast<const uint32_t *>(w), bias, y, B, H, W, Ho, Wo, Cd);
    RFD_HIP(hipGetLastError());
    return RFD_OK;
}

__global__ void __launch_bounds__(256) dwconv3x3_kernel(const bf16_t *__restrict__ x, const bf16_t *__restrict__ w,
                                                        const float *__restrict__ bias, bf16_t *__restrict__ y, int B,
                                                        int H, int W, int C, int Ho, int Wo, int stride)
{
    const int cg = C >> 3;
    const long long total = (long long)B * Ho * Wo * cg;
    const long long i = (long long)blockIdx.x * 256 + threadIdx.x;
    if (i >= total) return;
    const int c = (int)(i % cg) * 8;
    long long pix = i / cg;
    const int wo = (int)(pix % Wo);
    pix /= Wo;
    const int ho = (int)(pix % Ho);
    const int b = (int)(pix / Ho);
    float acc[8];
    {
        const float4 b0 = *reinterpret_cast<const float4 *>(bias + c), b1 = *reinterpret_cast<const float4 *>(bias + c + 4);
        acc[0] = b0.x; acc[1] = b0.y; acc[2] = b0.z; acc[3] = b0.w; acc[4] = b1.x; acc[5] = b1.y; acc[6] = b1.z; acc[7] = b1.w;
    }
#pragma unroll
    for (int ky = 0; ky < 3; ++ky) {
        const int hi = ho * stride - 1 + ky;
        if ((unsigned)hi >= (unsigned)H) continue;
#pragma unroll
        for (int kx = 0; kx < 3; ++kx) {
            const int wi = wo * stride - 1 + kx;
            if ((unsigned)wi >= (unsigned)W) continue;
// ... 53 lines not shown
```

### rs-face-detection_amd/csrc/kernels_pre.hip

```cpp
#include "kernels.h"

namespace rfd {

__device__ __forceinline__ int coef11(float v)
{
    int r = __float2int_rn(v);
    return max(-32768, min(32767, r));
}

__device__ __forceinline__ void resize_linear_px(const uint8_t *src, long long stride, int h, int w, double scale_x,
                                                 double scale_y, int area_fast, int x, int y, int v[3])
{
    if (area_fast) {
        const uint8_t *s0 = src + (long long)(2 * y) * stride + 2 * x * 3;
        const uint8_t *s1 = s0 + stride;
#pragma unroll
        for (int c = 0; c < 3; ++c) v[c] = (s0[c] + s0[c + 3] + s1[c] + s1[c + 3] + 2) >> 2;
        return;
    }
    float fx = (float)(((double)x + 0.5) * scale_x - 0.5);
    int sx = (int)floorf(fx);
    fx -= (float)sx;
    if (sx < 0) { fx = 0.0f; sx = 0; }
    if (sx >= w - 1) { fx = 0.0f; sx = w - 1; }
    const int a0 = coef11((1.0f - fx) * 2048.0f), a1 = coef11(fx * 2048.0f);
    const int sx1 = min(sx + 1, w - 1);

    float fy = (float)(((double)y + 0.5) * scale_y - 0.5);
    const int sy = (int)floorf(fy);
    fy -= (float)sy;
    const int b0 = coef11((1.0f - fy) * 2048.0f), b1 = coef11(fy * 2048.0f);
    const int sy0 = min(max(sy, 0), h - 1), sy1 = min(max(sy + 1, 0), h - 1);
    const uint8_t *S0 = src + (long long)sy0 * stride;
    const uint8_t *S1 = src + (long long)sy1 * stride;
    typedef uint64_t u64_unaligned __attribute__((aligned(1)));
    int t0[6], t1[6];
    const long long o0 = (long long)sy0 * stride + sx * 3, o1 = (long long)sy1 * stride + sx * 3, lim = (long long)(h - 1) * stride + (long long)w * 3 - 8;
    if (sx1 == sx + 1 && o0 <= lim && o1 <= lim) {
        const uint64_t q0 = *reinterpret_cast<const u64_unaligned *>(src + o0), q1 = *reinterpret_cast<const u64_unaligned *>(src + o1);
#pragma unroll
        for (int k = 0; k < 6; ++k) { t0[k] = (int)((q0 >> (8 * k)) & 0xff); t1[k] = (int)((q1 >> (8 * k)) & 0xff); }
    } else {
#pragma unroll
        for (int c = 0; c < 3; ++c) { t0[c] = S0[sx * 3 + c]; t0[3 + c] = S0[sx1 * 3 + c]; t1[c] = S1[sx * 3 + c]; t1[3 + c] = S1[sx1 * 3 + c]; }
    }
#pragma unroll
    for (int c = 0; c < 3; ++c) {
        const int r0 = t0[c] * a0 + t0[3 + c] * a1;
        const int r1 = t1[c] * a0 + t1[3 + c] * a1;
        v[c] = (((b0 * (r0 >> 4)) >> 16) + ((b1 * (r1 >> 4)) >> 16) + 2) >> 2;
        v[c] = min(255, max(0, v[c]));
    }
}

__global__ void __launch_bounds__(256) preprocess_kernel(PreParams p)
{
    const int b = blockIdx.z;
    const int x = blockIdx.x * 64 + (threadIdx.x & 63);
    const int y = blockIdx.y * 4 + (threadIdx.x >> 6);
    if (x >= p.net_w || y >= p.net_h) return;
    const PreImage im = p.imgs[b];

    int v[3] = {0, 0, 0};
    if (x < im.new_w && y < im.new_h) resize_linear_px(im.src, im.stride, im.h, im.w, im.scale_x, im.scale_y, im.area_fast, x, y, v);
    const size_t pix = ((size_t)b * p.net_h + y) * p.net_w + x;
    if (p.out_nhwc4) {
        const uint32_t r = __float_as_uint((float)v[2]) >> 16, g = __float_as_uint((float)v[1]) >> 16;
        const uint32_t bl = __float_as_uint((float)v[0]) >> 16;
        uint2 o;
        o.x = r | (g << 16);
        o.y = bl;
        *reinterpret_cast<uint2 *>(p.out_nhwc4 + pix * 4) = o;
    }
    if (p.out_det_img) {
        uint8_t *d = p.out_det_img + pix * 3;
        d[0] = (uint8_t)v[0]; d[1] = (uint8_t)v[1]; d[2] = (uint8_t)v[2];
    }
    if (p.out_tensor) {
        const size_t plane = (size_t)p.net_h * p.net_w;
        float *t = p.out_tensor + (size_t)b * 3 * plane + (size_t)y * p.net_w + x;
        t[0] = ((float)v[2] / 1.0f - 0.0f) / 1.0f;
        t[plane] = ((float)v[1] / 1.0f - 0.0f) / 1.0f;
        t[2 * plane] = ((float)v[0] / 1.0f - 0.0f) / 1.0f;
    }
}

int launch_preprocess(const PreParams &p, int n, hipStream_t s)
{
    dim3 grid(ceil_div(p.net_w, 64), ceil_div(p.net_h, 4), n);
    hipLaunchKernelGGL(preprocess_kernel, grid, dim3(256), 0, s, p);
    RFD_HIP(hipGetLastError());
    return RFD_OK;
}

__device__ __forceinline__ uint32_t f32_to_bf16_bits(float f)
{
    uint32_t u = __float_as_uint(f);
    if ((u & 0x7fffffffu) > 0x7f800000u) return (u >> 16) | 0x40u;
    u += 0x7fffu + ((u >> 16) & 1u);
    return u >> 16;
}

__global__ void __launch_bounds__(256) tensor_to_nhwc4_kernel(const float *__restrict__ t,
                                                              bf16_t *__restrict__ out, size_t plane,
                                                              size_t total)
{
    const size_t i = (size_t)blockIdx.x * 256 + threadIdx.x;
    if (i >= total) return;
    const size_t b = i / plane, q = i - b * plane;
    const float *s = t + b * 3 * plane + q;
    uint2 o;
    o.x = f32_to_bf16_bits(s[0]) | (f32_to_bf16_bits(s[plane]) << 16);
    o.y = f32_to_bf16_bits(s[2 * plane]);
    *reinterpret_cast<uint2 *>(out + i * 4) = o;
}

int launch_tensor_to_nhwc4(const float *tensor, bf16_t *out, int n, int H, int W, hipStream_t s)
{
    const size_t plane = (size_t)H * W, total = plane * n;
    hipLaunchKernelGGL(tensor_to_nhwc4_kernel, dim3((unsigned)((total + 255) / 256)), dim3(256), 0, s,
                       tensor, out, plane, total);
    RFD_HIP(hipGetLastError());
    return RFD_OK;
}

constexpr int kLmedsIters = 13;

__device__ __forceinline__ unsigned cv_rng_next(unsigned long long &state)
{
    state = (unsigned long long)(unsigned)state * 4164903690u + (unsigned)(state >> 32);
    return (unsigned)state;
}

__device__ void similarity_2pt(const float *src, const float *dst, int i0, int i1, double M[6])
{
    const double x1 = src[2 * i0], y1 = src[2 * i0 + 1], x2 = src[2 * i1], y2 = src[2 * i1 + 1];
    const double X1 = dst[2 * i0], Y1 = dst[2 * i0 + 1], X2 = dst[2 * i1], Y2 = dst[2 * i1 + 1];
    const double d = 1. / ((x1 - x2) * (x1 - x2) + (y1 - y2) * (y1 - y2));
    const double S0 = d * ((X1 - X2) * (x1 - x2) + (Y1 - Y2) * (y1 - y2));
    const double S1 = d * ((Y1 - Y2) * (x1 - x2) - (X1 - X2) * (y1 - y2));
    const double S2 = d * ((Y1 - Y2) * (x1 * y2 - x2 * y1) - (X1 * y2 - X2 * y1) * (y1 - y2) - (X1 * x2 - X2 * x1) * (x1 - x2));
    const double S3 = d * (-(X1 - X2) * (x1 * y2 - x2 * y1) - (Y1 * x2 - Y2 * x1) * (x1 - x2) - (Y1 * y2 - Y2 * y1) * (y1 - y2));
    M[0] = S0; M[1] = -S1; M[2] = S2; M[3] = S1; M[4] = S0; M[5] = S3;
}

__device__ __forceinline__ void similarity_errors5(const float *src, const float *dst, const double M[6], float err[5])
{
    const float F0 = (float)M[0], F1 = (float)M[1], F2 = (float)M[2], F3 = (float)M[3], F4 = (float)M[4], F5 = (float)M[5];
#pragma unroll
    for (int i = 0; i < 5; ++i) {
        const float fx = src[2 * i], fy = src[2 * i + 1];
        const float a = F0 * fx + F1 * fy + F2 - dst[2 * i];
        const float b = F3 * fx + F4 * fy + F5 - dst[2 * i + 1];
        err[i] = a * a + b * b;
    }
}
// ... 292 lines not shown
```

### rs-face-detection_amd/csrc/network.h

```cpp
#pragma once
#include <string>
#include <vector>

#include "kernels.h"

namespace rfd {

enum LayerKind { LK_CONV = 0, LK_DEPTHWISE = 1, LK_FIRST3X3 = 2, LK_CONV0 = 3 };

struct Layer {
    std::string name;
    int cin, cout, kh, kw, stride, pad;
    int kind;
    int cin_d, cout_d;
    int has_affine;
    float gain;
    size_t w_off;
    size_t ldw;
    size_t w_elems;
    size_t b_off;
    size_t a_off;
};

enum OpKind { OP_CONV = 2, OP_STEM = 3, OP_DW = 4, OP_FIRST = 5, OP_B2B = 6 };

struct Op {
    int kind;
    int layer;
    int in, out, out2, outf, res;
    int in2, layer2;
    int in_affine;
    int layer_n2;
    int x_coff;
    int y_split, y_split_add;
    int n_valid;
    int branch;
    int layer_b, out_b;
    int relu, res_up2, res_post, head_softmax, y_coff;
};

struct TensorDesc {
    int C, H, W;
    int C_logical;
    int is_f32;
    int buffer;
    int first, last;
    size_t bytes_per_image() const { return (size_t)C * H * W * (is_f32 ? 4 : 2); }
};

struct Graph {
    int backbone = 0, net_h = 0, net_w = 0;
    std::vector<Layer> layers;
    std::vector<Op> ops;
    std::vector<TensorDesc> tensors;
    int input = -1;
    int heads[3] = {-1, -1, -1};
    size_t w_total = 0, b_total = 0, a_total = 0;
    std::vector<size_t> buffer_bytes_per_image;

    int build(int backbone, int net_w, int net_h);
    double macs_per_image() const;
    double layer_macs(int op_index) const;

  private:
    int add_tensor(int C, int H, int W, int f32 = 0);
    int add_layer(const std::string &name, int cin, int cout, int k, int stride, int pad, float gain,
                  int has_affine, int extra_k = 0, int parent = -1, int col_off = 0, int kind = LK_CONV,
                  int cout_dev = 0);
    int add_conv(int layer, int in, int out, int relu, int res = -1, int out2 = -1, int outf = -1);
    void build_r50();
    void build_mnet025();
    void plan();
};

struct OpLaunch {
    int kind;
    int force_tile;
    bool b2b_s1;
    ConvParams conv;
    B2BParams b2b;
    const bf16_t *x, *w;
    const float *bias, *scale, *shift;
    bf16_t *y;
    int B, H, W, C, stride;
    const bf16_t *w1;
    const float *bias1;
    bf16_t *t1;
};
int launch_op(const OpLaunch &l, hipStream_t s, bool *fused);
int op_kernels(const OpLaunch &l, int cus, std::string *names, bool *fused);

struct Network {
    Graph g;
    int max_batch = 0;
    bool weights_ready = false;
    bf16_t *d_w = nullptr;
    float *d_b = nullptr;
    bf16_t *d_zero = nullptr;
    int *d_fail = nullptr;
    std::vector<void *> d_buffers;
    bool profiling = false;
    int force_tile = 0;
    std::vector<hipEvent_t> ev;
    std::vector<float> op_ms;
    int prof_first = 0, prof_last = -1;

    int precision = 0;
    float *d_w32 = nullptr;
    void *d_stem32 = nullptr;
    std::vector<void *> d_buffers32;
    void *tensor_ptr32(int t, int batch_off = 0) const
    {
        if (g.tensors[t].is_f32 || t == g.input) return tensor_ptr(t, batch_off);
        const int bi = g.tensors[t].buffer;
        return (char *)d_buffers32[bi] + (size_t)batch_off * g.buffer_bytes_per_image[bi] * 2;
    }
    int run_f32(int B, hipStream_t s, int first_op, int last_op, int batch_off);
    int schedule = 0;
    float *d_sk_ws[3] = {nullptr, nullptr, nullptr};
    size_t sk_ws_bytes[3] = {0, 0, 0};
    unsigned *d_sk_cnt = nullptr;
    std::vector<int> sk_cnt_off, sk_cnt_n;
    bool latency_pass(int B) const { return schedule == RFD_SCHEDULE_LATENCY && precision == 0 && B >= 1 && B <= RFD_LATENCY_MAX_BATCH; }
    int create(int backbone, int net_w, int net_h, int max_batch, int precision = 0, int schedule = 0);
    void destroy();
    int init_synthetic(uint64_t seed, hipStream_t s);
    int get_layer(int idx, float *w, float *bias, hipStream_t s);
    int set_layer(int idx, const float *w, const float *bias, hipStream_t s);
    int get_affine(int idx, float *scale, float *shift, hipStream_t s);
    int set_affine(int idx, const float *scale, const float *shift, hipStream_t s);
    void *tensor_ptr(int t, int batch_off = 0) const
    {
        const int bi = g.tensors[t].buffer;
        void *base = (head_parity && bi < (int)d_alt.size() && d_alt[bi]) ? d_alt[bi] : d_buffers[bi];
        return (char *)base + (size_t)batch_off * g.buffer_bytes_per_image[bi];
    }
    std::vector<void *> d_alt;
    int head_parity = 0;
    int ensure_alt_heads();
    void op_launch(int i, int B, int batch_off, int part, bool offer_conv1, OpLaunch *out) const;
    int op_kernel_names(int n, int op, int cus, std::string *out) const;
    int plan_splitk();
    int run(int B, hipStream_t s, int first_op = 0, int last_op = -1, int batch_off = 0, int part = 0);
    int run_split(int B, hipStream_t s);
    int split_body(int B, hipStream_t s);
    int tune_streams(int B, int P, hipStream_t s);
    void assign_streams(int a, int b, int c);
    static constexpr int kPool = 8;
    hipStream_t pool[kPool] = {};
    bool tuned = false, tune = true;
    float tuned_ms = 0.f;
    int tuned_a = -1, tuned_b = -1;
    int run_graphed(int B, hipStream_t s);
    std::vector<hipGraphExec_t> graph_exec;
    std::vector<char> warmed;
    bool use_graph = true;
    static constexpr int kMaxParts = 4;
    hipStream_t side[kMaxParts][2] = {};
    hipEvent_t ev_fork[kMaxParts][2] = {}, ev_join[kMaxParts][2] = {};
    bool multi_stream = true;
    hipStream_t part_stream[kMaxParts] = {};
    hipEvent_t ev_part_fork = nullptr, ev_part_join[kMaxParts] = {};
    int co_running = 0;
    int split_min_part = 4;
    int split_max_parts = 2;
    int num_parts(int B) const
    {
        if (profiling || split_min_part < 1 || precision != 0 || latency_pass(B)) return 1;
        return std::max(1, std::min(std::min(split_max_parts, kMaxParts), B / split_min_part));
    }
    int pass_chains(int B, int *sizes) const
    {
        const int P = num_parts(B);
        for (int p = 0; p < P; ++p) sizes[p] = B / P + (p < B % P ? 1 : 0);
        return P;
    }
    int collect_profile();
};

}
```

### rs-face-detection_amd/csrc/network.hip

```cpp
#include "network.h"

#include <math.h>
#include <algorithm>
#include <utility>

namespace rfd {

int Graph::add_tensor(int C, int H, int W, int f32)
{
    TensorDesc t;
    t.C_logical = C;
    t.C = (f32 || C == 4 || C % 64 == 0) ? C : (C + 63) / 64 * 64;
    t.H = H; t.W = W; t.is_f32 = f32; t.buffer = -1; t.first = 1 << 30; t.last = -1;
    tensors.push_back(t);
    return (int)tensors.size() - 1;
}

int Graph::add_layer(const std::string &name, int cin, int cout, int k, int stride, int pad, float gain,
                     int has_affine, int extra_k, int parent, int col_off, int kind, int cout_dev)
{
    Layer L;
    L.name = name; L.cin = cin; L.cout = cout; L.kh = k; L.kw = k; L.stride = stride; L.pad = pad;
    L.gain = gain; L.has_affine = has_affine; L.kind = kind;
    L.cin_d = kind == LK_CONV ? (cin + 63) / 64 * 64 : cin;
// ... 611 lines not shown
        else if (L.kind == LK_FIRST3X3) { rows = L.cout; K = 36; }
        else if (L.kind == LK_DEPTHWISE) { rows = 9; K = L.cout_d; }
        std::vector<bf16_t> hw(rows * K);
        RFD_HIP(hipMemcpy2DAsync(hw.data(), K * sizeof(bf16_t), d_w + L.w_off, L.ldw * sizeof(bf16_t), K * sizeof(bf16_t), rows,
                                 hipMemcpyDeviceToHost, s));
        RFD_HIP(hipStreamSynchronize(s));
        if (L.kind == LK_CONV0) {
            for (int n = 0; n < L.cout; ++n)
                for (int ky = 0; ky < 7; ++ky)
                    for (int kx = 0; kx < 7; ++kx)
                        for (int c = 0; c < 3; ++c)
                            w[(((size_t)n * 7 + ky) * 7 + kx) * 3 + c] = bf16_to_f32_host(hw[((size_t)n * 7 + ky) * 32 + kx * 4 + c]);
        } else if (L.kind == LK_FIRST3X3) {
            for (int n = 0; n < L.cout; ++n)
                for (int t = 0; t < 9; ++t)
                    for (int c = 0; c < 3; ++c) w[((size_t)n * 9 + t) * 3 + c] = bf16_to_f32_host(hw[(size_t)n * 36 + t * 4 + c]);
        } else if (L.kind == LK_DEPTHWISE) {
            for (int c = 0; c < L.cout; ++c)
                for (int t = 0; t < 9; ++t) w[(size_t)c * 9 + t] = bf16_to_f32_host(hw[(size_t)t * K + c]);
        } else {
            for (int n = 0; n < L.cout; ++n)
                for (int t = 0; t < taps; ++t)
                    for (int c = 0; c < L.cin; ++c)
                        w[((size_t)n * taps + t) * L.cin + c] = bf16_to_f32_host(hw[(size_t)n * K + (size_t)t * L.cin_d + c]);
        }
    }
    if (bias) {
        RFD_HIP(hipMemcpyAsync(bias, d_b + L.b_off, L.cout * sizeof(float), hipMemcpyDeviceToHost, s));
        RFD_HIP(hipStreamSynchronize(s));
    }
    return RFD_OK;
}

int Network::set_affine(int idx, const float *scale, const float *shift, hipStream_t s)
{
    if (idx < 0 || idx >= (int)g.layers.size() || !g.layers[idx].has_affine) { set_error("layer %d has no affine", idx); return RFD_ERR_INVALID_ARG; }
    const Layer &L = g.layers[idx];
    RFD_HIP(hipMemcpyAsync(d_b + g.b_total + L.a_off, scale, L.cout * sizeof(float), hipMemcpyHostToDevice, s));
    RFD_HIP(hipMemcpyAsync(d_b + g.b_total + L.a_off + L.cout_d, shift, L.cout * sizeof(float), hipMemcpyHostToDevice, s));
    RFD_HIP(hipStreamSynchronize(s));
    return RFD_OK;
}

int Network::get_affine(int idx, float *scale, float *shift, hipStream_t s)
{
    if (idx < 0 || idx >= (int)g.layers.size() || !g.layers[idx].has_affine) { set_error("layer %d has no affine", idx); return RFD_ERR_INVALID_ARG; }
    const Layer &L = g.layers[idx];
    RFD_HIP(hipMemcpyAsync(scale, d_b + g.b_total + L.a_off, L.cout * sizeof(float), hipMemcpyDeviceToHost, s));
    RFD_HIP(hipMemcpyAsync(shift, d_b + g.b_total + L.a_off + L.cout_d, L.cout * sizeof(float), hipMemcpyDeviceToHost, s));
    RFD_HIP(hipStreamSynchronize(s));
    return RFD_OK;
}

void Network::op_launch(int i, int B, int batch_off, int part, bool offer_conv1, OpLaunch *out) const
{
    const Op &o = g.ops[i];
    const Layer &L = g.layers[o.layer];
    const TensorDesc &tin = g.tensors[o.in];
    OpLaunch &l = *out;
    memset(&l, 0, sizeof l);
    l.kind = o.kind;
    l.force_tile = force_tile;
    if (o.kind == OP_FIRST || o.kind == OP_DW || o.kind == OP_STEM) {
        l.x = (const bf16_t *)tensor_ptr(o.in, batch_off);
        l.w = d_w + L.w_off;
        l.bias = d_b + L.b_off;
        l.y = (bf16_t *)tensor_ptr(o.out, batch_off);
        l.B = B; l.H = tin.H; l.W = tin.W;
        l.C = o.kind == OP_FIRST ? g.tensors[o.out].C : tin.C;
        l.stride = L.stride;
    }
    if (o.kind == OP_STEM) {
        l.scale = d_b + g.b_total + L.a_off;
        l.shift = d_b + g.b_total + L.a_off + L.cout_d;
        if (offer_conv1 && i + 1 < (int)g.ops.size()) {
            const Op &n = g.ops[i + 1];
            const Layer &Ln = g.layers[n.layer];
            const bool plain = n.kind == OP_CONV && n.in == o.out && Ln.kh == 1 && Ln.kw == 1 && Ln.stride == 1 && Ln.cin_d == 64 &&
                               Ln.cout_d == 64 && n.relu && n.in_affine < 0 && n.res < 0 && n.layer2 < 0 && n.layer_n2 < 0 && n.out2 < 0 &&
                               n.outf < 0 && n.out >= 0 && n.x_coff == 0 && n.y_coff == 0 && n.branch == o.branch &&
                               g.tensors[n.out].C == 64 && n.n_valid >= 64 && n.y_split >= 64;
            if (plain) { l.w1 = d_w + Ln.w_off; l.bias1 = d_b + Ln.b_off; l.t1 = (bf16_t *)tensor_ptr(n.out, batch_off); }
        }
    } else if (o.kind == OP_B2B && L.cin_d == 64 && g.layers[o.layer_b].cout_d == 64) {
        l.b2b_s1 = true;
        B2BParams &bp = l.b2b;
        const Layer &Lb = g.layers[o.layer_b];
        bp.x = (const bf16_t *)tensor_ptr(o.in, batch_off);
        bp.w3 = d_w + L.w_off;
        bp.bias3 = d_b + L.b_off;
        if (o.layer2 >= 0) {
            const Layer &L2 = g.layers[o.layer2];
            bp.x2 = (const bf16_t *)tensor_ptr(o.in2, batch_off);
            bp.bias3b = d_b + L2.b_off;
            bp.Cin2 = L2.cin_d;
        }
        bp.res = o.res >= 0 ? (const bf16_t *)tensor_ptr(o.res, batch_off) : nullptr;
        bp.scale = d_b + g.b_total + L.a_off;
        bp.shift = d_b + g.b_total + L.a_off + L.cout_d;
        bp.raw = (bf16_t *)tensor_ptr(o.out, batch_off);
        bp.w1 = d_w + Lb.w_off;
        bp.bias1 = d_b + Lb.b_off;
        bp.t1 = (bf16_t *)tensor_ptr(o.out_b, batch_off);
        bp.B = B; bp.H = tin.H; bp.W = tin.W; bp.Cin = L.cin_d;
        bp.force_tile = force_tile;
    } else if (o.kind == OP_CONV || o.kind == OP_B2B) {
        const int tout = o.out >= 0 ? o.out : (o.out2 >= 0 ? o.out2 : o.outf);
        ConvParams &p = l.conv;
        p.x = (const bf16_t *)tensor_ptr(o.in, batch_off);
        p.w = d_w + L.w_off;
        p.bias = d_b + L.b_off;
        p.zero = d_zero;
        p.force_tile = force_tile;
        p.co_running = co_running;
        p.fail = d_fail;
        if (latency_pass(B) && !co_running && batch_off == 0 && part == 0 && !sk_cnt_n.empty()) {
            const int br = std::min(std::max(o.branch, 0), 2);
            p.latency = 1;
            p.sk_ws = d_sk_ws[br]; p.sk_ws_bytes = sk_ws_bytes[br];
            p.sk_cnt = d_sk_cnt + sk_cnt_off[i]; p.sk_cnt_n = sk_cnt_n[i];
        }
        p.res = o.res >= 0 ? (const bf16_t *)tensor_ptr(o.res, batch_off) : nullptr;
        if (o.layer2 >= 0) {
            const Layer &L2 = g.layers[o.layer2];
            const TensorDesc &t2 = g.tensors[o.in2];
            p.x2 = (const bf16_t *)tensor_ptr(o.in2, batch_off);
            p.bias2 = d_b + L2.b_off;
            p.H2 = t2.H; p.W2 = t2.W; p.Cin2 = L2.cin_d; p.stride2 = L2.stride;
        }
        if (o.in_affine >= 0) {
            const Layer &La = g.layers[o.in_affine];
            p.in_scale = d_b + g.b_total + La.a_off;
            p.in_shift = d_b + g.b_total + La.a_off + La.cout_d;
        }
        p.scale2 = d_b + g.b_total + L.a_off;
        p.shift2 = d_b + g.b_total + L.a_off + L.cout_d;
        p.y = o.out >= 0 ? (bf16_t *)tensor_ptr(o.out, batch_off) : nullptr;
        p.y2 = o.out2 >= 0 ? (bf16_t *)tensor_ptr(o.out2, batch_off) : nullptr;
        p.yf = o.outf >= 0 ? (float *)tensor_ptr(o.outf, batch_off) : nullptr;
        p.B = B; p.H = tin.H; p.W = tin.W; p.Cin = L.cin_d;
        p.Cout = L.cout_d + (o.layer_n2 >= 0 ? g.layers[o.layer_n2].cout_d : 0);
        p.n_valid = o.n_valid;
        p.ldx = tin.C; p.x_coff = o.x_coff; p.y_split = o.y_split; p.y_split_add = o.y_split_add;
        p.KH = L.kh; p.KW = L.kw; p.stride = L.stride; p.pad = L.pad;
        p.Ho = g.tensors[tout].H; p.Wo = g.tensors[tout].W;
        p.ldy = o.out >= 0 ? g.tensors[o.out].C : p.Cout;
        p.y_coff = o.y_coff;
        p.relu = o.relu; p.res_up2 = o.res_up2; p.res_post = o.res_post; p.head_softmax = o.head_softmax;
        if (o.kind == OP_B2B) {
            const Layer &Lb = g.layers[o.layer_b];
            p.w1 = d_w + Lb.w_off;
            p.bias1 = d_b + Lb.b_off;
            p.t1 = (bf16_t *)tensor_ptr(o.out_b, batch_off);
            p.n1 = Lb.cout_d;
        }
    }
}

int launch_op(const OpLaunch &l, hipStream_t s, bool *fused)
{
    *fused = false;
    switch (l.kind) {
    case OP_FIRST: return launch_first3x3(l.x, l.w, l.bias, l.y, l.B, l.H, l.W, l.C, s);
    case OP_DW: return launch_dwconv3x3(l.x, l.w, l.bias, l.y, l.B, l.H, l.W, l.C, l.stride, s);
    case OP_STEM: return launch_stem(l.x, l.w, l.bias, l.scale, l.shift, l.y, l.B, l.H, l.W, s, l.force_tile, l.w1, l.bias1, l.t1, l.w1 ? fused : nullptr);
    default: return l.b2b_s1 ? launch_conv_b2b_s1(l.b2b, s) : launch_conv(l.conv, s);
    }
}

int op_kernels(const OpLaunch &l, int cus, std::string *names, bool *fused)
{
    *fused = false;
    ConvPlan plan;
    plan.steps = 1;
    switch (l.kind) {
    case OP_FIRST: plan.step[0].kernel = K_FIRST3X3; break;
    case OP_DW: plan.step[0].kernel = K_DWCONV3X3; break;
    case OP_STEM:
        plan.step[0].kernel = choose_stem(l.B, l.H, l.W, l.w1 && l.t1, l.force_tile, cus);
        *fused = plan.step[0].kernel == K_STEM_PERSISTENT_CONV1;
        break;
    default:
        if (l.b2b_s1) choose_b2b_s1(l.b2b, bank_behind(l.b2b.w3, l.b2b.w1), &plan.step[0]);
        else RFD_TRY(choose_conv(l.conv, bank_behind(l.conv.w, l.conv.w1), &plan));
    }
    names->clear();
    for (int i = 0; i < plan.steps; ++i) {
        if (i) *names += " + ";
        *names += conv_kernel_name(plan.step[i].kernel);
    }
    return RFD_OK;
}

int Network::op_kernel_names(int n, int op, int cus, std::string *out) const
{
    OpLaunch l;
    bool fused = false;
    if (op > 0 && g.ops[op - 1].kind == OP_STEM) {
        std::string stem;
        op_launch(op - 1, n, 0, 0, true, &l);
        RFD_TRY(op_kernels(l, cus, &stem, &fused));
        if (fused) { *out = "(fused into " + stem + ")"; return RFD_OK; }
    }
    op_launch(op, n, 0, 0, g.ops[op].kind == OP_STEM, &l);
    return op_kernels(l, cus, out, &fused);
}

int Network::run(int B, hipStream_t s, int first_op, int last_op, int batch_off, int part)
{
    if (!weights_ready) { set_error("network weights are not initialised (rfd_init_synthetic_weights / rfd_set_layer_weights)"); return RFD_ERR_STATE; }
    if (B < 1 || batch_off + B > max_batch) { set_error("batch %d exceeds max_batch_size %d", batch_off + B, max_batch); return RFD_ERR_CAPACITY; }
    if (precision != 0) return run_f32(B, s, first_op, last_op, batch_off);
    const int nops = (int)g.ops.size();
    if (profiling && (int)ev.size() < 2 * nops) {
        const size_t old = ev.size();
        ev.resize(2 * nops);
        for (size_t i = old; i < ev.size(); ++i) RFD_HIP(hipEventCreate(&ev[i]));
    }
    if (last_op < 0 || last_op >= nops) last_op = nops - 1;
    if (part == 0) { prof_first = std::max(first_op, 0); prof_last = last_op; }
    hipStream_t main_stream = s;
    const bool fork_ok = multi_stream && !profiling && first_op <= 0 && last_op == nops - 1 && side[part][0] && side[part][1];
    bool forked[2] = {false, false};
#ifdef RFD_DIAG
    static const std::vector<int> skip_ops = [] {
        std::vector<int> v;
        if (const char *e = getenv("RFD_SKIP_OPS"))
            for (const char *q = e; *q;) { v.push_back(atoi(q)); while (*q && *q != ',') ++q; if (*q == ',') ++q; }
        return v;
    }();
#else
    static const std::vector<int> skip_ops;
#endif
    for (int i = std::max(first_op, 0); i <= last_op; ++i) {
        const Op &o = g.ops[i];
        s = main_stream;
        if (!skip_ops.empty() && std::find(skip_ops.begin(), skip_ops.end(), i) != skip_ops.end()) {
            if (profiling) { RFD_HIP(hipEventRecord(ev[2 * i], s)); RFD_HIP(hipEventRecord(ev[2 * i + 1], s)); }
            continue;
        }
        if (fork_ok && o.branch > 0) {
            const int bidx = o.branch - 1;
            if (!forked[bidx]) {
                RFD_HIP(hipEventRecord(ev_fork[part][bidx], main_stream));
                RFD_HIP(hipStreamWaitEvent(side[part][bidx], ev_fork[part][bidx], 0));
                forked[bidx] = true;
            }
            s = side[part][bidx];
        }
        if (profiling) RFD_HIP(hipEventRecord(ev[2 * i], s));
        OpLaunch L;
        op_launch(i, B, batch_off, part, !profiling && i + 1 <= last_op && skip_ops.empty(), &L);
        bool fused = false;
        RFD_TRY(launch_op(L, s, &fused));
        if (profiling) RFD_HIP(hipEventRecord(ev[2 * i + 1], s));
        if (fused) ++i;
    }
    for (int bidx = 0; bidx < 2; ++bidx)
        if (forked[bidx]) {
            RFD_HIP(hipEventRecord(ev_join[part][bidx], side[part][bidx]));
            RFD_HIP(hipStreamWaitEvent(main_stream, ev_join[part][bidx], 0));
        }
    return RFD_OK;
}

int Network::run_f32(int B, hipStream_t s, int first_op, int last_op, int batch_off)
{
    const int nops = (int)g.ops.size();
    if (last_op < 0 || last_op >= nops) last_op = nops - 1;
    const float *aff = d_b + g.b_total;
    for (int i = std::max(first_op, 0); i <= last_op; ++i) {
        const Op &o = g.ops[i];
        const Layer &L = g.layers[o.layer];
        const TensorDesc &tin = g.tensors[o.in];
        if (o.kind == OP_STEM) {
            const size_t need = (size_t)max_batch * (tin.H / 2) * (tin.W / 2) * 64 * sizeof(float);
            if (!d_stem32) RFD_HIP(hipMalloc(&d_stem32, need));
            float *c0 = (float *)d_stem32 + (size_t)batch_off * (tin.H / 2) * (tin.W / 2) * 64;
            RFD_TRY(launch_conv0_f32((const bf16_t *)tensor_ptr(o.in, batch_off), d_w32 + L.w_off, d_b + L.b_off, c0, B, tin.H, tin.W, s));
            RFD_TRY(launch_maxpool_f32(c0, (float *)tensor_ptr32(o.out, batch_off), aff + L.a_off, aff + L.a_off + L.cout_d, B, tin.H / 2,
                                       tin.W / 2, 64, s));
            continue;
        }
        if (o.kind != OP_CONV && o.kind != OP_B2B) { set_error("f32 parity mode: op kind %d has no f32 kernel", o.kind); return RFD_ERR_INVALID_ARG; }
        const int tout = o.out >= 0 ? o.out : (o.out2 >= 0 ? o.out2 : o.outf);
        ConvF32Params p;
        memset(&p, 0, sizeof p);
        p.x = (const float *)tensor_ptr32(o.in, batch_off);
// ... 92 lines not shown
    co_running = 1;
    int off = 0, st = RFD_OK;
    for (int p = 0; p < P && st == RFD_OK; ++p) {
        const int Bp = sizes[p];
        RFD_HIP(hipStreamWaitEvent(part_stream[p], ev_part_fork, 0));
        st = run(Bp, part_stream[p], 0, -1, off, p);
        if (st == RFD_OK) RFD_HIP(hipEventRecord(ev_part_join[p], part_stream[p]));
        off += Bp;
    }
    co_running = 0;
    RFD_TRY(st);
    for (int p = 0; p < P; ++p) RFD_HIP(hipStreamWaitEvent(s, ev_part_join[p], 0));
    return RFD_OK;
}

int Network::tune_streams(int B, int P, hipStream_t s)
{
    hipEvent_t e0 = nullptr, e1 = nullptr;
    RFD_HIP(hipEventCreate(&e0));
    RFD_HIP(hipEventCreate(&e1));
    int st = RFD_OK;
    auto time_set = [&](int a, int b, int c, int reps, float *out) {
        assign_streams(a, b, c);
        std::vector<float> ts;
        for (int rep = 0; rep <= reps && st == RFD_OK; ++rep) {
            if (hipEventRecord(e0, s) != hipSuccess) st = RFD_ERR_HIP;
            if (st == RFD_OK) st = split_body(B, s);
            if (st == RFD_OK && (hipEventRecord(e1, s) != hipSuccess || hipEventSynchronize(e1) != hipSuccess)) st = RFD_ERR_HIP;
            float ms = 0.f;
            if (st == RFD_OK && hipEventElapsedTime(&ms, e0, e1) == hipSuccess && rep > 0) ts.push_back(ms);
        }
        std::sort(ts.begin(), ts.end());
        *out = ts.empty() ? 1e30f : ts[ts.size() / 2];
    };
    struct Cand { float t; int a, b, c; };
    std::vector<Cand> cand;
    for (int a = 0; a < kPool && st == RFD_OK; ++a)
        for (int b = a + 1; b < kPool && st == RFD_OK; ++b) {
            if (P == 2) {
                float t;
                time_set(a, b, -1, 2, &t);
                cand.push_back({t, a, b, -1});
            } else {
                for (int c = b + 1; c < kPool && st == RFD_OK; ++c) {
                    float t;
                    time_set(a, b, c, 2, &t);
                    cand.push_back({t, a, b, c});
                }
            }
        }
    std::sort(cand.begin(), cand.end(), [](const Cand &x, const Cand &y) { return x.t < y.t; });
    float best = 1e30f;
    int ba = 2, bb = 5, bc = P == 3 ? 6 : -1;
    for (size_t i = 0; i < cand.size() && i < 4 && st == RFD_OK; ++i) {
        float t;
        time_set(cand[i].a, cand[i].b, cand[i].c, 9, &t);
        if (t < best) { best = t; ba = cand[i].a; bb = cand[i].b; bc = cand[i].c; }
    }
    (void)hipEventDestroy(e0);
    (void)hipEventDestroy(e1);
    RFD_TRY(st);
    assign_streams(ba, bb, bc);
    tuned_ms = best;
    tuned_a = ba; tuned_b = bb;
    if (getenv("RFD_STREAM_TUNE_VERBOSE")) fprintf(stderr, "[rfd] chain streams: pool[%d], pool[%d], pool[%d] (%.3f ms per split pass at B = %d)\n", ba, bb, bc, best, B);
    return RFD_OK;
}

int Network::run_split(int B, hipStream_t s)
{
    const int P = num_parts(B);
    co_running = 0;
    if (P <= 1) return run(B, s);
    if (!tuned && tune && (P == 2 || P == 3)) {
        tuned = true;
        if (getenv("RFD_STREAM_TUNE") && atoi(getenv("RFD_STREAM_TUNE")) == 0) return split_body(B, s);
        RFD_TRY(tune_streams(B, P, s));
    }
    return split_body(B, s);
}

int Network::run_graphed(int B, hipStream_t s)
{
    if (!use_graph || profiling || B < 1 || B > max_batch || num_parts(B) > 1) return run_split(B, s);
    if ((int)graph_exec.size() <= max_batch) { graph_exec.assign(max_batch + 1, nullptr); warmed.assign(max_batch + 1, 0); }
    if (graph_exec[B]) {
        RFD_HIP(hipGraphLaunch(graph_exec[B], s));
        return RFD_OK;
    }
    if (!warmed[B]) {
        warmed[B] = 1;
        return run_split(B, s);
    }
    hipGraph_t graph = nullptr;
    static const bool linear_graph = getenv("GPU_MAX_HW_QUEUES") && atoi(getenv("GPU_MAX_HW_QUEUES")) < 3;
    const bool ms_saved = multi_stream;
    if (linear_graph) multi_stream = false;
    RFD_HIP(hipStreamBeginCapture(s, hipStreamCaptureModeThreadLocal));
    const int st = run_split(B, s);
    const hipError_t e = hipStreamEndCapture(s, &graph);
    multi_stream = ms_saved;
    if (st != RFD_OK || e != hipSuccess || !graph) {
        if (graph) (void)hipGraphDestroy(graph);
        use_graph = false;
        return st != RFD_OK ? st : run_split(B, s);
    }
    hipGraphExec_t exec = nullptr;
    const hipError_t ei = hipGraphInstantiate(&exec, graph, nullptr, nullptr, 0);
    (void)hipGraphDestroy(graph);
    if (ei != hipSuccess || !exec) {
        use_graph = false;
        return run_split(B, s);
    }
    graph_exec[B] = exec;
    RFD_HIP(hipGraphLaunch(exec, s));
    return RFD_OK;
}

int Network::collect_profile()
{
    const int nops = (int)g.ops.size();
    op_ms.assign(nops, 0.f);
    if (!profiling || (int)ev.size() < 2 * nops) return RFD_OK;
    for (int i = prof_first; i <= prof_last && i < nops; ++i) RFD_HIP(hipEventElapsedTime(&op_ms[i], ev[2 * i], ev[2 * i + 1]));
    return RFD_OK;
}

}
```

### rs-face-detection_amd/python/rfd_hip/__init__.py

```python
import ctypes as C
import os

import numpy as np

_HERE = os.path.dirname(os.path.abspath(__file__))
LIB_PATH = os.path.normpath(os.path.join(_HERE, "..", "..", "librfd_hip.so"))

RFD_OK = 0
RFD_ERR_INVALID_ARG = -1
RFD_ERR_NO_DEVICE = -2
PRECISION_BF16, PRECISION_F32 = 0, 1
SCHEDULE_THROUGHPUT, SCHEDULE_LATENCY = 0, 1
LATENCY_MAX_BATCH = 2
RFD_ERR_HIP = -3
RFD_ERR_CAPACITY = -4
RFD_ERR_STATE = -5
RFD_ERR_IO = -6
RFD_ERR_COMM = -7
COMM_ID_BYTES = 128
MAX_FACE_TENSORS = 4

(TILE_HEURISTIC, TILE_128, TILE_256x128, TILE_256x64, TILE_NO_128, TILE_NO_PW_STREAM, TILE_PERSISTENT, TILE_GENERIC, TILE_PW_STREAM,
 TILE_C64, TILE_PW_STREAM_K128, TILE_PW_STREAM_K256, TILE_PW_WIDE, TILE_HALO_SMALL, TILE_HALO_LARGE, TILE_PW_GEMM, TILE_PAIR, TILE_RING,
 TILE_128_EIGHT_WAVES, TILE_KX_FOUR_WAVES) = range(20)
# ... 4 lines not shown
NUM_ANCHORS = 2


class RfdError(RuntimeError):
    def __init__(self, status, message):
        super().__init__("rfd status %d: %s" % (status, message))
        self.status = status


class rfd_config(C.Structure):
    _fields_ = [("image_w", C.c_int), ("image_h", C.c_int), ("max_batch_size", C.c_int),
                ("confidence_threshold", C.c_float), ("iou_threshold", C.c_float),
                ("device_id", C.c_int), ("max_det", C.c_int), ("max_src_w", C.c_int),
                ("max_src_h", C.c_int), ("backbone", C.c_int), ("precision", C.c_int), ("schedule", C.c_int),
                ("reserved", C.c_int * 4)]


class rfd_image(C.Structure):
    _fields_ = [("data", C.c_void_p), ("height", C.c_int), ("width", C.c_int),
                ("stride", C.c_ssize_t)]


class rfd_dets(C.Structure):
    _fields_ = [("boxes", C.c_void_p), ("landmarks", C.c_void_p), ("count", C.c_void_p),
                ("total", C.c_void_p)]


class rfd_stats(C.Structure):
    _fields_ = [("ms_h2d", C.c_float), ("ms_preprocess", C.c_float), ("ms_network", C.c_float),
                ("ms_decode", C.c_float), ("ms_sort", C.c_float), ("ms_nms", C.c_float),
                ("ms_d2h", C.c_float), ("ms_total", C.c_float), ("candidates", C.c_int64),
                ("detections", C.c_int64), ("reserved", C.c_int64 * 4)]

    def as_dict(self):
        return {k: getattr(self, k) for k, _ in self._fields_ if k != "reserved"}


class rfd_layer_desc(C.Structure):
    _fields_ = [("name", C.c_char * 64), ("cin", C.c_int), ("cout", C.c_int), ("kh", C.c_int),
                ("kw", C.c_int), ("stride", C.c_int), ("pad", C.c_int), ("has_affine", C.c_int),
                ("kind", C.c_int), ("reserved", C.c_int * 3)]


class rfd_op_desc(C.Structure):
    _fields_ = [("kind", C.c_int), ("layer", C.c_int), ("in_", C.c_int), ("out", C.c_int),
                ("out2", C.c_int), ("outf", C.c_int), ("res", C.c_int), ("relu", C.c_int),
                ("res_up2", C.c_int), ("res_post", C.c_int), ("head_softmax", C.c_int),
                ("y_coff", C.c_int), ("macs", C.c_double), ("in2", C.c_int), ("layer2", C.c_int),
                ("in_affine", C.c_int), ("layer_n2", C.c_int), ("x_coff", C.c_int), ("y_split", C.c_int),
                ("y_split_add", C.c_int), ("n_valid", C.c_int), ("branch", C.c_int), ("layer_b", C.c_int),
                ("out_b", C.c_int)]


class rfd_alignment_config(C.Structure):
    _fields_ = [("out_w", C.c_int32), ("out_h", C.c_int32), ("standard_landmarks", C.c_float * 10),
                ("reserved", C.c_int32 * 4)]


class rfd_face_tensor_config(C.Structure):
    _fields_ = [("out_w", C.c_int32), ("out_h", C.c_int32), ("mean", C.c_float * 3), ("scale", C.c_float * 3),
                ("reserved", C.c_int32 * 4)]


class rfd_faces(C.Structure):
    _fields_ = [("box", C.c_void_p), ("kps", C.c_void_p), ("found", C.c_void_p), ("crops", C.c_void_p),
                ("status", C.c_void_p), ("tensors", C.c_void_p * MAX_FACE_TENSORS)]


class rfd_tensor_desc(C.Structure):
    _fields_ = [("channels", C.c_int), ("height", C.c_int), ("width", C.c_int),
                ("is_f32", C.c_int), ("buffer", C.c_int), ("is_input", C.c_int),
                ("head_level", C.c_int), ("channels_logical", C.c_int), ("reserved", C.c_int * 3)]


API_SYMBOLS = [
    "rfd_config_default", "rfd_create", "rfd_destroy", "rfd_last_error", "rfd_version",
    "rfd_graph_create", "rfd_graph_destroy", "rfd_graph_counts", "rfd_graph_layer", "rfd_graph_op",
    "rfd_graph_tensor", "rfd_graph_macs", "rfd_graph_workspace_bytes",
    "rfd_init_synthetic_weights", "rfd_num_layers", "rfd_get_layer_weights",
    "rfd_set_layer_weights", "rfd_get_layer_affine", "rfd_set_layer_affine", "rfd_detect_batch",
    "rfd_detect_batch_device", "rfd_sync", "rfd_set_stream", "rfd_preprocess", "rfd_forward", "rfd_decode_nms",
    "rfd_nms_sorted", "_nms", "rfd_get_stats", "rfd_get_config", "rfd_set_thresholds", "rfd_set_profiling",
    "rfd_get_conv_profile", "rfd_get_op_profile", "rfd_debug_tensor_io", "rfd_debug_run_ops", "rfd_debug_run_chain", "rfd_debug_pass_chains", "rfd_debug_buffer_io",
    "rfd_debug_set_conv_tile", "rfd_debug_op_kernels", "rfd_debug_op_kernels_static", "rfd_debug_set_concurrency", "rfd_debug_persistent_kernel", "rfd_debug_poke_nms_flag", "rfd_selection_config_default",
    "rfd_select_faces", "rfd_detect_select_batch", "rfd_save_weights", "rfd_load_weights",
    "rfd_alignment_config_default", "rfd_align_faces", "rfd_detect_select_align_batch",
    "rfd_host_alloc", "rfd_host_free", "rfd_submit_batch", "rfd_collect_batch",
    "rfd_comm_get_unique_id", "rfd_comm_init", "rfd_comm_info", "rfd_gather_detections", "rfd_comm_destroy",
    "rfd_face_tensor_config_quality", "rfd_face_tensor_config_extraction", "rfd_face_tensors",
    "rfd_align_faces_tensors", "rfd_detect_select_align_tensors_batch", "rfd_detect_faces_device", "rfd_quality_decide", "rfd_normalize_embeddings",
    "rfd_quality_decide_device", "rfd_normalize_embeddings_device",
]

_lib = None


def load_library(path=None):
    global _lib
    if _lib is not None and path is None:
        return _lib
    p = path or os.environ.get("RFD_HIP_LIB") or LIB_PATH
    if not os.path.exists(p):
        raise ImportError("librfd_hip.so not found at %s -- build it with "
                          "rs-face-detection_amd/build.sh (there is no CPU fallback)" % p)
    L = C.CDLL(p)
    vp, ci = C.c_void_p, C.c_int
    L.rfd_last_error.restype = C.c_char_p
    L.rfd_config_default.argtypes = [C.POINTER(rfd_config)]
    L.rfd_config_default.restype = None
    L.rfd_create.argtypes = [C.POINTER(rfd_config), C.POINTER(vp)]
    L.rfd_destroy.argtypes = [vp]
    L.rfd_destroy.restype = None
    L.rfd_graph_create.argtypes = [ci, ci, ci, C.POINTER(vp)]
    L.rfd_graph_destroy.argtypes = [vp]
    L.rfd_graph_destroy.restype = None
    L.rfd_graph_counts.argtypes = [vp] + [C.POINTER(ci)] * 4
    L.rfd_graph_layer.argtypes = [vp, ci, C.POINTER(rfd_layer_desc)]
    L.rfd_graph_op.argtypes = [vp, ci, C.POINTER(rfd_op_desc)]
    L.rfd_graph_tensor.argtypes = [vp, ci, C.POINTER(rfd_tensor_desc)]
    L.rfd_graph_macs.argtypes = [vp]
    L.rfd_graph_macs.restype = C.c_double
    L.rfd_graph_workspace_bytes.argtypes = [vp]
    L.rfd_graph_workspace_bytes.restype = C.c_double
    L.rfd_init_synthetic_weights.argtypes = [vp, C.c_uint64]
    L.rfd_num_layers.argtypes = [vp]
    L.rfd_get_layer_weights.argtypes = [vp, ci, vp, vp]
    L.rfd_set_layer_weights.argtypes = [vp, ci, vp, vp]
    L.rfd_get_layer_affine.argtypes = [vp, ci, vp, vp]
    L.rfd_set_layer_affine.argtypes = [vp, ci, vp, vp]
    L.rfd_detect_batch.argtypes = [vp, C.POINTER(rfd_image), ci, C.POINTER(rfd_dets)]
    L.rfd_detect_batch_device.argtypes = [vp, C.POINTER(rfd_image), ci, C.POINTER(rfd_dets), ci]
    L.rfd_sync.argtypes = [vp]
    L.rfd_set_stream.argtypes = [vp, vp]
    L.rfd_preprocess.argtypes = [vp, C.POINTER(rfd_image), ci, vp, vp, vp]
    L.rfd_forward.argtypes = [vp, vp, ci, C.POINTER(vp)]
    L.rfd_decode_nms.argtypes = [vp, C.POINTER(vp), ci, vp, C.POINTER(rfd_dets), vp]
    L.rfd_nms_sorted.argtypes = [vp, vp, C.POINTER(ci), vp, ci, ci, C.c_float]
    L._nms.argtypes = [vp, C.POINTER(ci), vp, ci, ci, C.c_float, ci]
    L._nms.restype = None
    L.rfd_get_stats.argtypes = [vp, C.POINTER(rfd_stats)]
    L.rfd_get_config.argtypes = [vp, C.POINTER(rfd_config)]
    L.rfd_set_thresholds.argtypes = [vp, C.c_float, C.c_float]
    L.rfd_set_profiling.argtypes = [vp, ci]
    L.rfd_get_conv_profile.argtypes = [vp, C.POINTER(C.c_float), C.POINTER(C.c_double), C.POINTER(ci)]
    L.rfd_get_op_profile.argtypes = [vp, vp, ci]
    L.rfd_debug_tensor_io.argtypes = [vp, ci, ci, vp, ci]
    L.rfd_debug_run_ops.argtypes = [vp, ci, ci, ci]
    L.rfd_debug_run_chain.argtypes = [vp, ci, ci, ci, ci, ci]
    L.rfd_debug_pass_chains.argtypes = [vp, ci, C.POINTER(ci), ci]
    L.rfd_debug_buffer_io.argtypes = [vp, ci, vp, C.c_size_t, ci, C.POINTER(C.c_size_t)]
    L.rfd_debug_set_conv_tile.argtypes = [vp, ci]
    L.rfd_debug_set_concurrency.argtypes = [vp, ci, ci, ci, ci]
    L.rfd_debug_op_kernels.argtypes = [vp, ci, ci, ci, C.c_char_p, ci]
    L.rfd_debug_op_kernels_static.argtypes = [ci] * 9 + [C.c_char_p, ci]
    L.rfd_debug_poke_nms_flag.argtypes = [vp, ci]
    L.rfd_debug_persistent_kernel.argtypes = [ci, C.POINTER(C.c_char_p), C.POINTER(C.c_size_t)]
    L.rfd_save_weights.argtypes = [vp, C.c_char_p]
    L.rfd_load_weights.argtypes = [vp, C.c_char_p]
    L.rfd_selection_config_default.argtypes = [vp]
    L.rfd_selection_config_default.restype = None
    L.rfd_select_faces.argtypes = [vp, C.POINTER(rfd_dets), vp, vp, ci, vp, ci, vp, vp, vp]
    L.rfd_detect_select_batch.argtypes = [vp, C.POINTER(rfd_image), ci, vp, ci, vp, vp, vp]
    L.rfd_host_alloc.argtypes = [C.c_size_t, C.POINTER(C.c_void_p)]
    L.rfd_host_free.argtypes = [vp]
    L.rfd_submit_batch.argtypes = [vp, C.POINTER(rfd_image), ci]
    L.rfd_collect_batch.argtypes = [vp, C.POINTER(rfd_dets), C.POINTER(ci)]
    L.rfd_comm_get_unique_id.argtypes = [vp]
    L.rfd_comm_init.argtypes = [vp, vp, ci, ci]
    L.rfd_comm_info.argtypes = [vp, C.POINTER(ci), C.POINTER(ci)]
    L.rfd_gather_detections.argtypes = [vp, C.POINTER(rfd_dets), ci, C.POINTER(rfd_dets)]
    L.rfd_comm_destroy.argtypes = [vp]
    L.rfd_alignment_config_default.argtypes = [C.POINTER(rfd_alignment_config)]
    L.rfd_alignment_config_default.restype = None
    L.rfd_align_faces.argtypes = [vp, C.POINTER(rfd_image), ci, vp, vp, vp, vp, vp, vp]
    L.rfd_detect_select_align_batch.argtypes = [vp, C.POINTER(rfd_image), ci, vp, ci, vp, vp, vp, vp, vp, vp]
    for f in (L.rfd_face_tensor_config_quality, L.rfd_face_tensor_config_extraction):
        f.argtypes = [C.POINTER(rfd_face_tensor_config)]
        f.restype = None
    L.rfd_face_tensors.argtypes = [vp, vp, ci, ci, ci, vp, ci, C.POINTER(vp)]
    L.rfd_detect_select_align_tensors_batch.argtypes = [vp, C.POINTER(rfd_image), ci, vp, ci, vp, vp, vp, vp, vp, vp, vp, ci, C.POINTER(vp)]
    L.rfd_align_faces_tensors.argtypes = [vp, C.POINTER(rfd_image), ci, vp, vp, vp, vp, vp, vp, vp, ci, C.POINTER(vp)]
    L.rfd_detect_faces_device.argtypes = [vp, C.POINTER(rfd_image), ci, vp, ci, vp, vp, ci, C.POINTER(rfd_faces), ci]
    L.rfd_quality_decide.argtypes = [vp, vp, ci, ci, C.c_float, vp, vp]
    L.rfd_quality_decide_device.argtypes = [vp, vp, ci, ci, C.c_float, vp, vp]
    L.rfd_normalize_embeddings.argtypes = [vp, vp, ci, ci, vp]
    L.rfd_normalize_embeddings_device.argtypes = [vp, vp, ci, ci, vp]
    if path is None:
        _lib = L
    return L


def _check(status):
    if status < 0:
        raise RfdError(status, load_library().rfd_last_error().decode("utf-8", "replace"))
    return status


def face_tensor_config(image_size, mean, scale):
    c = rfd_face_tensor_config()
    c.out_w, c.out_h = int(image_size[0]), int(image_size[1])
    for i in range(3):
        c.mean[i], c.scale[i] = mean[i], scale[i]
    return c


def face_tensor_config_quality():
    c = rfd_face_tensor_config()
    load_library().rfd_face_tensor_config_quality(C.byref(c))
    return c


def face_tensor_config_extraction():
    c = rfd_face_tensor_config()
    load_library().rfd_face_tensor_config_extraction(C.byref(c))
    return c


def _face_tensor_args(cfgs, n):
    k = len(cfgs)
    arr = (rfd_face_tensor_config * max(k, 1))(*cfgs)
    outs = [np.zeros((n, 3, max(c.out_h, 1), max(c.out_w, 1)), np.float32) for c in cfgs]
    ptrs = (C.c_void_p * max(k, 1))(*[o.ctypes.data for o in outs])
    return arr, outs, ptrs


def op_kernels_static(backbone, image_w, image_h, n, op, co_running=True, tile=0, schedule=SCHEDULE_THROUGHPUT, cus=256):
    buf = C.create_string_buffer(512)
    _check(load_library().rfd_debug_op_kernels_static(backbone, image_w, image_h, n, op, 1 if co_running else 0, tile, schedule, cus, buf, 512))
    return buf.value.decode().split(" + ")


def head_shapes(n, net_h, net_w):
    out = []
    for s in STRIDES:
        h, w = net_h // s, net_w // s
        out += [(n, 2 * NUM_ANCHORS, h, w), (n, 4 * NUM_ANCHORS, h, w), (n, 10 * NUM_ANCHORS, h, w)]
    return out

# ... 347 lines not shown
        assert x.ndim == 2
        score, klass = np.zeros(x.shape[0], np.float32), np.zeros(x.shape[0], np.int32)
        _check(self._L.rfd_quality_decide(self._ctx, x.ctypes.data, x.shape[0], x.shape[1], float(threshold), score.ctypes.data,
                                          klass.ctypes.data))
        return score, klass

    def normalize_embeddings(self, emb):
        x = np.ascontiguousarray(emb, np.float32)
        assert x.ndim == 2
        out = np.zeros_like(x)
        _check(self._L.rfd_normalize_embeddings(self._ctx, x.ctypes.data, x.shape[0], x.shape[1], out.ctypes.data))
        return out

    def preprocess(self, frames):
        arr, keep = self._images(frames)
        n = len(frames)
        w, h = self.image_size
        det_img = np.zeros((n, h, w, 3), np.uint8)
        tensor = np.zeros((n, 3, h, w), np.float32)
        scale = np.zeros(n, np.float32)
        _check(self._L.rfd_preprocess(self._ctx, arr, n, det_img.ctypes.data, tensor.ctypes.data,
                                      scale.ctypes.data))
        return det_img, tensor, scale

    def forward(self, tensor):
        t = np.ascontiguousarray(tensor, np.float32)
        n = t.shape[0]
        w, h = self.image_size
        assert t.shape == (n, 3, h, w)
        heads = [np.zeros(s, np.float32) for s in head_shapes(n, h, w)]
        ptrs = (C.c_void_p * 9)(*[x.ctypes.data for x in heads])
        _check(self._L.rfd_forward(self._ctx, t.ctypes.data, n, ptrs))
        return heads

    def decode_nms(self, heads, det_scale, want_gidx=False):
        hs = [np.ascontiguousarray(x, np.float32) for x in heads]
        n = hs[0].shape[0]
        w, h = self.image_size
        for x, s in zip(hs, head_shapes(n, h, w)):
            if x.shape != s:
                raise RfdError(RFD_ERR_INVALID_ARG, "head shape %s != %s" % (x.shape, s))
        sc = np.ascontiguousarray(det_scale, np.float32).reshape(n)
        ptrs = (C.c_void_p * 9)(*[x.ctypes.data for x in hs])
        d, boxes, lmk, count, total = self._alloc_dets(n)
        gidx = np.zeros((n, self.max_det), np.int32)
        _check(self._L.rfd_decode_nms(self._ctx, ptrs, n, sc.ctypes.data, C.byref(d),
                                      gidx.ctypes.data if want_gidx else None))
        self.last_total = total
        res = self._split(boxes, lmk, count)
        if want_gidx:
            res = [(a, b, gidx[i, :count[i]].copy()) for i, (a, b) in enumerate(res)]
        return res

    def nms_sorted(self, boxes, thresh):
        b = np.ascontiguousarray(boxes, np.float32)
        keep = np.zeros(max(b.shape[0], 1), np.int32)
        num = C.c_int(0)
        _check(self._L.rfd_nms_sorted(self._ctx, keep.ctypes.data, C.byref(num), b.ctypes.data,
                                      b.shape[0], b.shape[1] if b.ndim == 2 else 5, float(thresh)))
        return keep[:num.value].copy()

    def debug_write(self, tensor_id, arr):
        a = np.ascontiguousarray(arr)
        _check(self._L.rfd_debug_tensor_io(self._ctx, tensor_id, a.shape[0], a.ctypes.data, 1))

    def debug_read(self, tensor_id, n, desc):
        dt = np.float32 if desc.is_f32 else np.uint16
        a = np.zeros((n, desc.height, desc.width, desc.channels), dt)
        _check(self._L.rfd_debug_tensor_io(self._ctx, tensor_id, n, a.ctypes.data, 0))
        return a

    def debug_set_conv_tile(self, tile):
        _check(self._L.rfd_debug_set_conv_tile(self._ctx, tile))

    def debug_op_kernels(self, n, op, co_running=True):
        buf = C.create_string_buffer(512)
        _check(self._L.rfd_debug_op_kernels(self._ctx, n, op, 1 if co_running else 0, buf, 512))
        return buf.value.decode().split(" + ")

    def debug_set_concurrency(self, multi_stream=True, split_min_part=8, split_max_parts=2, use_graph=True):
        _check(self._L.rfd_debug_set_concurrency(self._ctx, int(multi_stream), int(split_min_part), int(split_max_parts),
                                                 int(use_graph)))

    def debug_run(self, n, first_op, last_op, batch_off=0, co_running=False):
        if batch_off == 0 and not co_running:
            _check(self._L.rfd_debug_run_ops(self._ctx, n, first_op, last_op))
        else:
            _check(self._L.rfd_debug_run_chain(self._ctx, n, first_op, last_op, batch_off, 1 if co_running else 0))

    def debug_pass_chains(self, n):
        sizes = (C.c_int * 8)()
        return list(sizes[:_check(self._L.rfd_debug_pass_chains(self._ctx, n, sizes, 8))])

    def debug_buffer_pitch(self, tensor_id):
        pitch = C.c_size_t()
        _check(self._L.rfd_debug_buffer_io(self._ctx, tensor_id, None, 0, 0, C.byref(pitch)))
        return pitch.value

    def debug_buffer_read(self, tensor_id):
        a = np.zeros(self.cfg.max_batch_size * self.debug_buffer_pitch(tensor_id), np.uint8)
        _check(self._L.rfd_debug_buffer_io(self._ctx, tensor_id, a.ctypes.data, a.nbytes, 0, None))
        return a

    def debug_buffer_write(self, tensor_id, arr):
        a = np.ascontiguousarray(arr).reshape(-1).view(np.uint8)
        _check(self._L.rfd_debug_buffer_io(self._ctx, tensor_id, a.ctypes.data, a.nbytes, 1, None))

    def stats(self):
        s = rfd_stats()
        _check(self._L.rfd_get_stats(self._ctx, C.byref(s)))
        return s.as_dict()

    def set_thresholds(self, confidence_threshold, iou_threshold):
        _check(self._L.rfd_set_thresholds(self._ctx, confidence_threshold, iou_threshold))

    def set_profiling(self, enable):
        _check(self._L.rfd_set_profiling(self._ctx, 1 if enable else 0))

    def conv_profile(self):
        ms, fl, n = C.c_float(), C.c_double(), C.c_int()
        _check(self._L.rfd_get_conv_profile(self._ctx, C.byref(ms), C.byref(fl), C.byref(n)))
        return ms.value, fl.value, n.value

    def op_profile(self, nops):
        ms = np.zeros(nops, np.float32)
        _check(self._L.rfd_get_op_profile(self._ctx, ms.ctypes.data, nops))
        return ms
```

Before: 8288 images/s.

## Fuse letterbox resize preprocessing into the persistent stem convolution loader

The persistent stem kernel can now read raw uint8 frames directly, doing the bilinear/area resize and letterbox conversion while loading its input patch. This skips the separate preprocess kernel and the bf16 NHWC4 input tensor write and read. Fusion applies only when the stem chooses a persistent variant and the frames are large enough for wide loads; otherwise the old preprocess path runs. The stem now keeps twice the prefetch registers and recomputes resize addresses per tile, and the eager (ungraphed) path is taken when fusion is on.

```diff
diff --git a/include/rfd.h b/include/rfd.h
--- a/include/rfd.h
+++ b/include/rfd.h
@@ -250,6 +250,8 @@
                                         int cus, char *names, int cap);
 RFD_API int rfd_debug_set_concurrency(rfd_ctx *ctx, int multi_stream, int split_min_part, int split_max_parts,
                                       int use_graph);
+RFD_API int rfd_debug_set_fused_preprocess(rfd_ctx *ctx, int on);
+RFD_API int rfd_debug_run_chain_from_frames(rfd_ctx *ctx, const rfd_image *imgs, int n, int last_op, int batch_off);
 
 RFD_API int rfd_debug_poke_nms_flag(rfd_ctx *ctx, int value);
 RFD_API int rfd_debug_persistent_kernel(int i, const char **name, size_t *lds_bytes);
diff --git a/rs-face-detection_amd/csrc/detector.hip b/rs-face-detection_amd/csrc/detector.hip
--- a/rs-face-detection_amd/csrc/detector.hip
+++ b/rs-face-detection_amd/csrc/detector.hip
@@ -204,6 +204,7 @@
     Rccl::Comm comm = nullptr;
     int comm_rank = 0, comm_world = 0;
     rfd_stats stats;
+    bool pre_fused = false;
     float conv_ms = 0.f;
     double conv_flops = 0.0;
     int conv_launches = 0;
@@ -366,7 +367,7 @@
     float ms;
     memset(&c->stats, 0, sizeof c->stats);
     auto el = [&](int a, int b) { return hipEventElapsedTime(&ms, c->ev[a], c->ev[b]) == hipSuccess ? ms : 0.f; };
-    if (have_pre) { c->stats.ms_h2d = el(0, 1); c->stats.ms_preprocess = el(1, 2); }
+    if (have_pre) { c->stats.ms_h2d = el(0, 1); c->stats.ms_preprocess = c->pre_fused ? 0.f : el(1, 2); }
     if (have_net) c->stats.ms_network = el(2, 3);
     c->stats.ms_decode = el(3, 4);
     c->stats.ms_sort = el(4, 5);
@@ -387,6 +388,39 @@
             }
     }
     return RFD_OK;
+}
+
+bool frames_take_wide_loads(const rfd_image *imgs, int n)
+{
+    for (int i = 0; i < n; ++i)
+        if ((long long)imgs[i].height * imgs[i].width * 3 < 8) return false;
+    return true;
+}
+
+int pass_input(rfd_ctx *c, const rfd_image *imgs, const PreImage *d_imgs, int n, hipStream_t s, bool *pre_ran = nullptr)
+{
+    Network &net = c->net;
+    int chain[Network::kMaxParts];
+    const int P = net.pass_chains(n, chain);
+    const bool eager = net.pass_is_eager(n);
+    const size_t in_px = (size_t)c->cfg.image_h * c->cfg.image_w * 4;
+    if (pre_ran) *pre_ran = false;
+    for (int p = 0, off = 0; p < P; off += chain[p], ++p) {
+        net.src_imgs[p] = nullptr;
+        if (eager && net.stem_reads_source(chain[p]) && frames_take_wide_loads(imgs + off, chain[p])) { net.src_imgs[p] = d_imgs + off; continue; }
+        if (pre_ran) *pre_ran = true;
+        PreParams pp;
+        memset(&pp, 0, sizeof pp);
+        pp.imgs = d_imgs + off;
+        pp.net_h = c->cfg.image_h; pp.net_w = c->cfg.image_w;
+        pp.out_nhwc4 = (bf16_t *)net.tensor_ptr(net.g.input) + (size_t)off * in_px;
+        RFD_TRY(launch_preprocess(pp, chain[p], s));
+    }
+    return RFD_OK;
+}
+void pass_input_done(rfd_ctx *c)
+{
+    for (int p = 0; p < Network::kMaxParts; ++p) c->net.src_imgs[p] = nullptr;
 }
 
 int detect_overlapped(rfd_ctx *c, const rfd_image *imgs, int n, rfd_dets *out, hipEvent_t frames_ready = nullptr)
@@ -442,13 +476,18 @@
     int status = RFD_OK;
     for (int p = 0; p < 2 && status == RFD_OK; ++p) {
         const int off = p ? B0 : 0, Bp = chain[p];
-        PreParams pp;
-        memset(&pp, 0, sizeof pp);
-        pp.imgs = (const PreImage *)c->ov_imgs[par].p + off;
-        pp.net_h = c->cfg.image_h; pp.net_w = c->cfg.image_w;
-        pp.out_nhwc4 = (bf16_t *)net.tensor_ptr(net.g.input) + (size_t)off * in_px;
-        status = launch_preprocess(pp, Bp, st[p]);
+        const bool from_frames = net.stem_reads_source(Bp) && frames_take_wide_loads(imgs + off, Bp);
+        if (!from_frames) {
+            PreParams pp;
+            memset(&pp, 0, sizeof pp);
+            pp.imgs = (const PreImage *)c->ov_imgs[par].p + off;
+            pp.net_h = c->cfg.image_h; pp.net_w = c->cfg.image_w;
+            pp.out_nhwc4 = (bf16_t *)net.tensor_ptr(net.g.input) + (size_t)off * in_px;
+            status = launch_preprocess(pp, Bp, st[p]);
+        }
+        net.src_imgs[p] = from_frames ? (const PreImage *)c->ov_imgs[par].p + off : nullptr;
         if (status == RFD_OK) status = net.run(Bp, st[p], 0, -1, off, p);
+        net.src_imgs[p] = nullptr;
         if (status == RFD_OK && hipEventRecord(c->ov_chain_done[par][p], st[p]) != hipSuccess) status = RFD_ERR_HIP;
     }
     net.co_running = 0;
@@ -482,14 +521,13 @@
     RFD_HIP(hipEventRecord(c->ev[0], c->stream));
     RFD_TRY(stage_frames(c, imgs, n, frames_on_device, scales));
     RFD_HIP(hipEventRecord(c->ev[1], c->stream));
-    PreParams pp;
-    memset(&pp, 0, sizeof pp);
-    pp.imgs = (const PreImage *)c->imgs.p;
-    pp.net_h = c->cfg.image_h; pp.net_w = c->cfg.image_w;
-    pp.out_nhwc4 = (bf16_t *)c->net.tensor_ptr(c->net.g.input);
-    RFD_TRY(launch_preprocess(pp, n, c->stream));
+    bool pre_ran = true;
+    RFD_TRY(pass_input(c, imgs, (const PreImage *)c->imgs.p, n, c->stream, &pre_ran));
+    c->pre_fused = !pre_ran;
     RFD_HIP(hipEventRecord(c->ev[2], c->stream));
-    RFD_TRY(c->net.run_graphed(n, c->stream));
+    const int net_status = c->net.run_graphed(n, c->stream);
+    pass_input_done(c);
+    RFD_TRY(net_status);
     RFD_HIP(hipEventRecord(c->ev[3], c->stream));
     DecodeParams dp;
     fill_decode_params(c, dp);
@@ -826,6 +864,13 @@
         if (ge) { (void)hipGraphExecDestroy(ge); ge = nullptr; }
     return RFD_OK;
 }
+int rfd_debug_set_fused_preprocess(rfd_ctx *c, int on)
+{
+    RFD_CHECK_ARG(c, "ctx is null");
+    RFD_TRY(c->ensure_network());
+    c->net.fused_pre = on != 0;
+    return RFD_OK;
+}
 int rfd_debug_poke_nms_flag(rfd_ctx *c, int value)
 {
     RFD_CHECK_ARG(c, "ctx is null");
@@ -865,6 +910,35 @@
     RFD_HIP(hipStreamSynchronize(c->stream));
     if (c->net.profiling) RFD_TRY(c->net.collect_profile());
     return check_nms_flag(c);
+}
+int rfd_debug_run_chain_from_frames(rfd_ctx *c, const rfd_image *imgs, int n, int last_op, int batch_off)
+{
+    RFD_CHECK_ARG(c, "ctx is null");
+    RFD_TRY(check_images(c, imgs, n));
+    RFD_HIP(hipSetDevice(c->cfg.device_id));
+    RFD_TRY(c->ensure_network());
+    RFD_CHECK_ARG(batch_off >= 0 && batch_off + n <= c->cfg.max_batch_size, "chain [batch_off, batch_off + n) out of range");
+    Network &net = c->net;
+    c->ov_last_n = -1;
+    std::vector<float> scales;
+    RFD_TRY(stage_frames(c, imgs, n, true, scales));
+    const bool from_frames = net.stem_reads_source(n) && frames_take_wide_loads(imgs, n);
+    if (!from_frames) {
+        PreParams pp;
+        memset(&pp, 0, sizeof pp);
+        pp.imgs = (const PreImage *)c->imgs.p;
+        pp.net_h = c->cfg.image_h; pp.net_w = c->cfg.image_w;
+        pp.out_nhwc4 = (bf16_t *)net.tensor_ptr(net.g.input, batch_off);
+        RFD_TRY(launch_preprocess(pp, n, c->stream));
+    }
+    net.src_imgs[0] = from_frames ? (const PreImage *)c->imgs.p : nullptr;
+    const int st = net.run(n, c->stream, 0, last_op, batch_off, 0);
+    net.src_imgs[0] = nullptr;
+    RFD_TRY(st);
+    RFD_HIP(hipMemcpyAsync(c->h_nms_flag, net.d_fail, sizeof(int), hipMemcpyDeviceToHost, c->stream));
+    RFD_HIP(hipStreamSynchronize(c->stream));
+    RFD_TRY(check_nms_flag(c));
+    return from_frames ? 1 : 0;
 }
 int rfd_debug_pass_chains(rfd_ctx *c, int n, int *sizes, int cap)
 {
@@ -1229,13 +1303,10 @@
     } else {
         c->ov_last_n = -1;
         RFD_HIP(hipStreamWaitEvent(c->stream, ps.h2d, 0));
-        PreParams pp;
-        memset(&pp, 0, sizeof pp);
-        pp.imgs = (const PreImage *)ps.imgs.p;
-        pp.net_h = c->cfg.image_h; pp.net_w = c->cfg.image_w;
-        pp.out_nhwc4 = (bf16_t *)c->net.tensor_ptr(c->net.g.input);
-        RFD_TRY(launch_preprocess(pp, n, c->stream));
-        RFD_TRY(c->net.run_graphed(n, c->stream));
+        RFD_TRY(pass_input(c, imgs, (const PreImage *)ps.imgs.p, n, c->stream));
+        const int net_status = c->net.run_graphed(n, c->stream);
+        pass_input_done(c);
+        RFD_TRY(net_status);
         DecodeParams dp;
         fill_decode_params(c, dp);
         for (int l = 0; l < kNumLevels; ++l) dp.cls[l] = (const float *)c->net.tensor_ptr(c->net.g.heads[l]);
diff --git a/rs-face-detection_amd/csrc/kernels.h b/rs-face-detection_amd/csrc/kernels.h
--- a/rs-face-detection_amd/csrc/kernels.h
+++ b/rs-face-detection_amd/csrc/kernels.h
@@ -304,7 +304,7 @@
 ConvKernel choose_stem(int B, int H, int W, bool conv1_offered, int force_tile, int cus);
 int launch_stem(const bf16_t *x4, const bf16_t *w, const float *bias, const float *scale, const float *shift,
                 bf16_t *y, int B, int H, int W, hipStream_t s, int force_tile = 0, const bf16_t *w1 = nullptr,
-                const float *bias1 = nullptr, bf16_t *t1 = nullptr, bool *fused = nullptr);
+                const float *bias1 = nullptr, bf16_t *t1 = nullptr, bool *fused = nullptr, const PreImage *pre_imgs = nullptr);
 int launch_first3x3(const bf16_t *x4, const bf16_t *w, const float *bias, bf16_t *y, int B, int H, int W, int Cd,
                     hipStream_t s);
 int launch_dwconv3x3(const bf16_t *x, const bf16_t *w, const float *bias, bf16_t *y, int B, int H, int W, int C,
diff --git a/rs-face-detection_amd/csrc/kernels_conv.hip b/rs-face-detection_amd/csrc/kernels_conv.hip
--- a/rs-face-detection_amd/csrc/kernels_conv.hip
+++ b/rs-face-detection_amd/csrc/kernels_conv.hip
@@ -1,4 +1,5 @@
 #include "conv_device.h"
+#include "pre_device.h"
 
 namespace rfd {
 
@@ -2584,7 +2585,7 @@
                                                               const float *__restrict__ shift, bf16_t *__restrict__ y, int H,
                                                               int W, int tiles_w, int tiles_h, int ntiles, int per,
                                                               const bf16_t *__restrict__ w1, const float *__restrict__ bias1,
-                                                              bf16_t *__restrict__ t1)
+                                                              bf16_t *__restrict__ t1, const PreImage *__restrict__ pre_imgs)
 {
     RFD_CLOCK(12);
     __shared__ __attribute__((aligned(16))) uint2 in_tile[kStemIR * kStemIP];
@@ -2596,9 +2597,28 @@
     const int t_begin = (int)blockIdx.x * per, t_end = min(ntiles, t_begin + per);
     if (t_begin >= t_end) return;
     constexpr int NR = (kStemIR * kStemIP + 255) / 256;
-    auto load_patch = [&](int t, uint2 (&pre)[NR]) {
-        const int tw_ = t % tiles_w, th_ = (t / tiles_w) % tiles_h, b_ = t / (tiles_w * tiles_h);
-        const int ir0_ = 2 * (2 * th_ * kStemPH - 1) - 3, ic0_ = 2 * (2 * tw_ * kStemPW - 1) - 3;
+    auto patch_origin = [&](int t, int &b_, int &ir0_, int &ic0_) {
+        const int tw_ = t % tiles_w, th_ = (t / tiles_w) % tiles_h;
+        b_ = t / (tiles_w * tiles_h);
+        ir0_ = 2 * (2 * th_ * kStemPH - 1) - 3; ic0_ = 2 * (2 * tw_ * kStemPW - 1) - 3;
+    };
+    auto load_patch = [&](int t, uint4 (&pre)[NR]) {
+        int b_, ir0_, ic0_;
+        patch_origin(t, b_, ir0_, ic0_);
+        if (pre_imgs) {
+            const PreImage im = pre_imgs[b_];
+#pragma unroll
+            for (int round = 0; round < NR; ++round) {
+                const int i = tid + round * 256;
+                const int r = i / kStemIP, c = i - r * kStemIP;
+                const int gr = ir0_ + r, gc = ic0_ + c;
+                const bool ok = c < kStemIC && (unsigned)gr < (unsigned)H && (unsigned)gc < (unsigned)W && letterbox_inside(im, gc, gr);
+                const ResizeAddr a = resize_linear_addr(im.stride, im.h, im.w, im.scale_x, im.scale_y, im.area_fast, ok ? gc : 0, ok ? gr : 0);
+                const ResizeTaps tp = resize_linear_load<true>(im.src, a);
+                pre[round] = make_uint4((uint32_t)tp.q0, (uint32_t)(tp.q0 >> 32), (uint32_t)tp.q1, (uint32_t)(tp.q1 >> 32));
+            }
+            return;
+        }
         const uint2 *src_ = reinterpret_cast<const uint2 *>(x4) + (size_t)b_ * H * W;
 #pragma unroll
         for (int round = 0; round < NR; ++round) {
@@ -2608,14 +2628,35 @@
             const bool ok = c < kStemIC && (unsigned)gr < (unsigned)H && (unsigned)gc < (unsigned)W;
             const uint32_t keep = ok ? 0xffffffffu : 0u;
             const uint2 v = src_[ok ? (size_t)gr * W + gc : (size_t)0];
-            pre[round] = make_uint2(v.x & keep, v.y & keep);
+            pre[round] = make_uint4(v.x & keep, v.y & keep, 0u, 0u);
         }
     };
-    auto store_patch = [&](const uint2 (&pre)[NR]) {
+    auto store_patch = [&](int t, const uint4 (&pre)[NR]) {
+        if (pre_imgs) {
+            int b_, ir0_, ic0_;
+            patch_origin(t, b_, ir0_, ic0_);
+            const PreImage im = pre_imgs[b_];
+#pragma unroll
+            for (int round = 0; round < NR; ++round) {
+                const int i = tid + round * 256;
+                const int r = i / kStemIP, c = i - r * kStemIP;
+                const int gr = ir0_ + r, gc = ic0_ + c;
+                const bool ok = c < kStemIC && (unsigned)gr < (unsigned)H && (unsigned)gc < (unsigned)W && letterbox_inside(im, gc, gr);
+                const uint32_t keep = ok ? 0xffffffffu : 0u;
+                ResizeTaps tp;
+                tp.q0 = (uint64_t)pre[round].x | ((uint64_t)pre[round].y << 32);
+                tp.q1 = (uint64_t)pre[round].z | ((uint64_t)pre[round].w << 32);
+                int v[3];
+                resize_linear_finish(im.stride, im.h, im.w, im.scale_x, im.scale_y, im.area_fast, ok ? gc : 0, ok ? gr : 0, tp, v);
+                const uint2 o = letterbox_nhwc4(v);
+                if (i < kStemIR * kStemIP) in_tile[i] = make_uint2(o.x & keep, o.y & keep);
+            }
+            return;
+        }
 #pragma unroll
         for (int round = 0; round < NR; ++round) {
             const int i = tid + round * 256;
-            if (i < kStemIR * kStemIP) in_tile[i] = pre[round];
+            if (i < kStemIR * kStemIP) in_tile[i] = make_uint2(pre[round].x, pre[round].y);
         }
     };
 
@@ -2627,9 +2668,9 @@
         for (int k = 0; k < 7; ++k)
             af[i][k] = *reinterpret_cast<const bf16x8 *>(w + ((size_t)chn * 7 + k) * 32 + fq * 8);
     }
-    uint2 pre[NR];
+    uint4 pre[NR];
     load_patch(t_begin, pre);
-    store_patch(pre);
+    store_patch(t_begin, pre);
     if (FUSE1) {
 #pragma unroll
         for (int round = 0; round < 2; ++round) {
@@ -2687,7 +2728,7 @@
         }
     }
         __syncthreads();
-        if (more) store_patch(pre);
+        if (more) store_patch(tile + 1, pre);
     static_assert(kStemPH * kStemPW * 8 % 256 == 0, "the pooling pass runs whole rounds of the workgroup (a scalar trip count)");
     static_assert(!FUSE1 || (kStemPW == 16 && kStemPH == 4), "fused conv1: a wave owns one pooled row of 16 pixels");
     uint4 yq[2];
@@ -2759,7 +2800,8 @@
 
 
 int launch_stem(const bf16_t *x4, const bf16_t *w, const float *bias, const float *scale, const float *shift,
-                bf16_t *y, int B, int H, int W, hipStream_t s, int force_tile, const bf16_t *w1, const float *bias1, bf16_t *t1, bool *fused)
+                bf16_t *y, int B, int H, int W, hipStream_t s, int force_tile, const bf16_t *w1, const float *bias1, bf16_t *t1, bool *fused,
+                const PreImage *pre_imgs)
 {
     if (fused) *fused = false;
     if ((H | W) & 3) {
@@ -2771,13 +2813,18 @@
     const int ntiles = B * tiles_h * tiles_w;
     const int slots = 2 * device_cus();
     const int per = ceil_div(ntiles, slots), grid = ceil_div(ntiles, per);
-    switch (choose_stem(B, H, W, w1 && t1 && fused, force_tile, device_cus())) {
+    const ConvKernel k = choose_stem(B, H, W, w1 && t1 && fused, force_tile, device_cus());
+    if (pre_imgs && k == K_STEM) {
+        set_error("stem: %d images run the one-tile kernel, which has no source-reading loader", B);
+        return RFD_ERR_STATE;
+    }
+    switch (k) {
     case K_STEM_PERSISTENT_CONV1:
         *fused = true;
-        hipLaunchKernelGGL(stem_persistent_kernel<true>, dim3((unsigned)grid), dim3(256), 0, s, x4, w, bias, scale, shift, y, H, W, tiles_w, tiles_h, ntiles, per, w1, bias1, t1);
+        hipLaunchKernelGGL(stem_persistent_kernel<true>, dim3((unsigned)grid), dim3(256), 0, s, x4, w, bias, scale, shift, y, H, W, tiles_w, tiles_h, ntiles, per, w1, bias1, t1, pre_imgs);
         break;
     case K_STEM_PERSISTENT:
-        hipLaunchKernelGGL(stem_persistent_kernel<false>, dim3((unsigned)grid), dim3(256), 0, s, x4, w, bias, scale, shift, y, H, W, tiles_w, tiles_h, ntiles, per, nullptr, nullptr, nullptr);
+        hipLaunchKernelGGL(stem_persistent_kernel<false>, dim3((unsigned)grid), dim3(256), 0, s, x4, w, bias, scale, shift, y, H, W, tiles_w, tiles_h, ntiles, per, nullptr, nullptr, nullptr, pre_imgs);
         break;
     default:
         hipLaunchKernelGGL(stem_kernel, dim3((unsigned)ntiles), dim3(256), 0, s, x4, w, bias, scale, shift, y,
diff --git a/rs-face-detection_amd/csrc/kernels_pre.hip b/rs-face-detection_amd/csrc/kernels_pre.hip
--- a/rs-face-detection_amd/csrc/kernels_pre.hip
+++ b/rs-face-detection_amd/csrc/kernels_pre.hip
@@ -1,57 +1,7 @@
 #include "kernels.h"
+#include "pre_device.h"
 
 namespace rfd {
-
-__device__ __forceinline__ int coef11(float v)
-{
-    int r = __float2int_rn(v);
-    return max(-32768, min(32767, r));
-}
-
-__device__ __forceinline__ void resize_linear_px(const uint8_t *src, long long stride, int h, int w, double scale_x,
-                                                 double scale_y, int area_fast, int x, int y, int v[3])
-{
-    if (area_fast) {
-        const uint8_t *s0 = src + (long long)(2 * y) * stride + 2 * x * 3;
-        const uint8_t *s1 = s0 + stride;
-#pragma unroll
-        for (int c = 0; c < 3; ++c) v[c] = (s0[c] + s0[c + 3] + s1[c] + s1[c + 3] + 2) >> 2;
-        return;
-    }
-    float fx = (float)(((double)x + 0.5) * scale_x - 0.5);
-    int sx = (int)floorf(fx);
-    fx -= (float)sx;
-    if (sx < 0) { fx = 0.0f; sx = 0; }
-    if (sx >= w - 1) { fx = 0.0f; sx = w - 1; }
-    const int a0 = coef11((1.0f - fx) * 2048.0f), a1 = coef11(fx * 2048.0f);
-    const int sx1 = min(sx + 1, w - 1);
-
-    float fy = (float)(((double)y + 0.5) * scale_y - 0.5);
-    const int sy = (int)floorf(fy);
-    fy -= (float)sy;
-    const int b0 = coef11((1.0f - fy) * 2048.0f), b1 = coef11(fy * 2048.0f);
-    const int sy0 = min(max(sy, 0), h - 1), sy1 = min(max(sy + 1, 0), h - 1);
-    const uint8_t *S0 = src + (long long)sy0 * stride;
-    const uint8_t *S1 = src + (long long)sy1 * stride;
-    typedef uint64_t u64_unaligned __attribute__((aligned(1)));
-    int t0[6], t1[6];
-    const long long o0 = (long long)sy0 * stride + sx * 3, o1 = (long long)sy1 * stride + sx * 3, lim = (long long)(h - 1) * stride + (long long)w * 3 - 8;
-    if (sx1 == sx + 1 && o0 <= lim && o1 <= lim) {
-        const uint64_t q0 = *reinterpret_cast<const u64_unaligned *>(src + o0), q1 = *reinterpret_cast<const u64_unaligned *>(src + o1);
-#pragma unroll
-        for (int k = 0; k < 6; ++k) { t0[k] = (int)((q0 >> (8 * k)) & 0xff); t1[k] = (int)((q1 >> (8 * k)) & 0xff); }
-    } else {
-#pragma unroll
-        for (int c = 0; c < 3; ++c) { t0[c] = S0[sx * 3 + c]; t0[3 + c] = S0[sx1 * 3 + c]; t1[c] = S1[sx * 3 + c]; t1[3 + c] = S1[sx1 * 3 + c]; }
-    }
-#pragma unroll
-    for (int c = 0; c < 3; ++c) {
-        const int r0 = t0[c] * a0 + t0[3 + c] * a1;
-        const int r1 = t1[c] * a0 + t1[3 + c] * a1;
-        v[c] = (((b0 * (r0 >> 4)) >> 16) + ((b1 * (r1 >> 4)) >> 16) + 2) >> 2;
-        v[c] = min(255, max(0, v[c]));
-    }
-}
 
 __global__ void __launch_bounds__(256) preprocess_kernel(PreParams p)
 {
@@ -62,16 +12,9 @@
     const PreImage im = p.imgs[b];
 
     int v[3] = {0, 0, 0};
-    if (x < im.new_w && y < im.new_h) resize_linear_px(im.src, im.stride, im.h, im.w, im.scale_x, im.scale_y, im.area_fast, x, y, v);
+    if (letterbox_inside(im, x, y)) resize_linear_px(im.src, im.stride, im.h, im.w, im.scale_x, im.scale_y, im.area_fast, x, y, v);
     const size_t pix = ((size_t)b * p.net_h + y) * p.net_w + x;
-    if (p.out_nhwc4) {
-        const uint32_t r = __float_as_uint((float)v[2]) >> 16, g = __float_as_uint((float)v[1]) >> 16;
-        const uint32_t bl = __float_as_uint((float)v[0]) >> 16;
-        uint2 o;
-        o.x = r | (g << 16);
-        o.y = bl;
-        *reinterpret_cast<uint2 *>(p.out_nhwc4 + pix * 4) = o;
-    }
+    if (p.out_nhwc4) *reinterpret_cast<uint2 *>(p.out_nhwc4 + pix * 4) = letterbox_nhwc4(v);
     if (p.out_det_img) {
         uint8_t *d = p.out_det_img + pix * 3;
         d[0] = (uint8_t)v[0]; d[1] = (uint8_t)v[1]; d[2] = (uint8_t)v[2];
diff --git a/rs-face-detection_amd/csrc/network.h b/rs-face-detection_amd/csrc/network.h
--- a/rs-face-detection_amd/csrc/network.h
+++ b/rs-face-detection_amd/csrc/network.h
@@ -84,6 +84,7 @@
     bf16_t *y;
     int B, H, W, C, stride;
     const bf16_t *w1;
+    const PreImage *pre_imgs;
     const float *bias1;
     bf16_t *t1;
 };
@@ -164,6 +165,10 @@
     int co_running = 0;
     int split_min_part = 4;
     int split_max_parts = 2;
+    bool pass_is_eager(int B) const { return !use_graph || profiling || B < 1 || B > max_batch || num_parts(B) > 1; }
+    bool fused_pre = true;
+    const PreImage *src_imgs[4] = {nullptr, nullptr, nullptr, nullptr};
+    bool stem_reads_source(int B) const;
     int num_parts(int B) const
     {
         if (profiling || split_min_part < 1 || precision != 0 || latency_pass(B)) return 1;
diff --git a/rs-face-detection_amd/csrc/network.hip b/rs-face-detection_amd/csrc/network.hip
--- a/rs-face-detection_amd/csrc/network.hip
+++ b/rs-face-detection_amd/csrc/network.hip
@@ -717,6 +717,7 @@
                                g.tensors[n.out].C == 64 && n.n_valid >= 64 && n.y_split >= 64;
             if (plain) { l.w1 = d_w + Ln.w_off; l.bias1 = d_b + Ln.b_off; l.t1 = (bf16_t *)tensor_ptr(n.out, batch_off); }
         }
+        if (o.in == g.input && part >= 0 && part < kMaxParts) l.pre_imgs = src_imgs[part];
     } else if (o.kind == OP_B2B && L.cin_d == 64 && g.layers[o.layer_b].cout_d == 64) {
         l.b2b_s1 = true;
         B2BParams &bp = l.b2b;
@@ -798,7 +799,7 @@
     switch (l.kind) {
     case OP_FIRST: return launch_first3x3(l.x, l.w, l.bias, l.y, l.B, l.H, l.W, l.C, s);
     case OP_DW: return launch_dwconv3x3(l.x, l.w, l.bias, l.y, l.B, l.H, l.W, l.C, l.stride, s);
-    case OP_STEM: return launch_stem(l.x, l.w, l.bias, l.scale, l.shift, l.y, l.B, l.H, l.W, s, l.force_tile, l.w1, l.bias1, l.t1, l.w1 ? fused : nullptr);
+    case OP_STEM: return launch_stem(l.x, l.w, l.bias, l.scale, l.shift, l.y, l.B, l.H, l.W, s, l.force_tile, l.w1, l.bias1, l.t1, l.w1 ? fused : nullptr, l.pre_imgs);
     default: return l.b2b_s1 ? launch_conv_b2b_s1(l.b2b, s) : launch_conv(l.conv, s);
     }
 }
@@ -839,6 +840,13 @@
     }
     op_launch(op, n, 0, 0, g.ops[op].kind == OP_STEM, &l);
     return op_kernels(l, cus, out, &fused);
+}
+
+bool Network::stem_reads_source(int B) const
+{
+    if (!fused_pre || precision != 0 || profiling || g.ops.empty() || g.ops[0].kind != OP_STEM || g.ops[0].in != g.input) return false;
+    const TensorDesc &tin = g.tensors[g.input];
+    return choose_stem(B, tin.H, tin.W, false, force_tile, device_cus()) != K_STEM;
 }
 
 int Network::run(int B, hipStream_t s, int first_op, int last_op, int batch_off, int part)
@@ -1097,7 +1105,7 @@
 
 int Network::run_graphed(int B, hipStream_t s)
 {
-    if (!use_graph || profiling || B < 1 || B > max_batch || num_parts(B) > 1) return run_split(B, s);
+    if (pass_is_eager(B)) return run_split(B, s);
     if ((int)graph_exec.size() <= max_batch) { graph_exec.assign(max_batch + 1, nullptr); warmed.assign(max_batch + 1, 0); }
     if (graph_exec[B]) {
         RFD_HIP(hipGraphLaunch(graph_exec[B], s));
diff --git a/rs-face-detection_amd/csrc/pre_device.h b/rs-face-detection_amd/csrc/pre_device.h
--- /dev/null
+++ b/rs-face-detection_amd/csrc/pre_device.h
@@ -0,0 +1,135 @@
+#pragma once
+#include "kernels.h"
+
+namespace rfd {
+
+__device__ __forceinline__ int coef11(float v)
+{
+    int r = __float2int_rn(v);
+    return max(-32768, min(32767, r));
+}
+
+struct ResizeTaps {
+    uint64_t q0, q1;
+};
+struct ResizeAddr {
+    long long c0, c1;
+    int sh0, sh1;
+    int d;
+};
+
+__device__ __forceinline__ void resize_linear_x(int w, double scale_x, int x, int &sx, float &fx)
+{
+    fx = (float)(((double)x + 0.5) * scale_x - 0.5);
+    sx = (int)floorf(fx);
+    fx -= (float)sx;
+    if (sx < 0) { fx = 0.0f; sx = 0; }
+    if (sx >= w - 1) { fx = 0.0f; sx = w - 1; }
+}
+__device__ __forceinline__ void resize_linear_y(double scale_y, int y, int &sy, float &fy)
+{
+    fy = (float)(((double)y + 0.5) * scale_y - 0.5);
+    sy = (int)floorf(fy);
+    fy -= (float)sy;
+}
+
+__device__ __forceinline__ bool resize_wide_ok(long long stride, int h, int w) { return (long long)(h - 1) * stride + (long long)w * 3 >= 8; }
+
+__device__ __forceinline__ ResizeAddr resize_linear_addr(long long stride, int h, int w, double scale_x, double scale_y, int area_fast,
+                                                         int x, int y)
+{
+    long long o0, o1;
+    ResizeAddr a;
+    if (area_fast) {
+        o0 = (long long)(2 * y) * stride + 2 * x * 3;
+        o1 = o0 + stride;
+        a.d = 3;
+    } else {
+        int sx, sy;
+        float fx, fy;
+        resize_linear_x(w, scale_x, x, sx, fx);
+        resize_linear_y(scale_y, y, sy, fy);
+        const int sx1 = min(sx + 1, w - 1);
+        const int sy0 = min(max(sy, 0), h - 1), sy1 = min(max(sy + 1, 0), h - 1);
+        o0 = (long long)sy0 * stride + sx * 3;
+        o1 = (long long)sy1 * stride + sx * 3;
+        a.d = (sx1 - sx) * 3;
+    }
+    const long long lim = (long long)(h - 1) * stride + (long long)w * 3 - 8;
+    a.c0 = lim >= 0 ? min(o0, lim) : o0;
+    a.c1 = lim >= 0 ? min(o1, lim) : o1;
+    a.sh0 = 8 * (int)(o0 - a.c0);
+    a.sh1 = 8 * (int)(o1 - a.c1);
+    return a;
+}
+
+template <bool WIDE>
+__device__ __forceinline__ ResizeTaps resize_linear_load(const uint8_t *src, const ResizeAddr &a)
+{
+    typedef const __attribute__((address_space(1))) uint8_t *global_u8_ptr;
+    typedef const __attribute__((address_space(1), aligned(1))) uint64_t *global_u64_unaligned_ptr;
+    const global_u8_ptr g = (global_u8_ptr)src;
+    ResizeTaps t;
+    if (WIDE) {
+        t.q0 = *(global_u64_unaligned_ptr)(g + a.c0);
+        t.q1 = *(global_u64_unaligned_ptr)(g + a.c1);
+    } else {
+        t.q0 = t.q1 = 0;
+#pragma unroll
+        for (int c = 0; c < 3; ++c) {
+            t.q0 |= ((uint64_t)g[a.c0 + c] << (8 * c)) | ((uint64_t)g[a.c0 + a.d + c] << (8 * (3 + c)));
+            t.q1 |= ((uint64_t)g[a.c1 + c] << (8 * c)) | ((uint64_t)g[a.c1 + a.d + c] << (8 * (3 + c)));
+        }
+    }
+    return t;
+}
+
+__device__ __forceinline__ void resize_linear_finish(long long stride, int h, int w, double scale_x, double scale_y, int area_fast, int x,
+                                                     int y, const ResizeTaps &t, int v[3])
+{
+    const ResizeAddr a = resize_linear_addr(stride, h, w, scale_x, scale_y, area_fast, x, y);
+    uint64_t q0 = t.q0 >> a.sh0, q1 = t.q1 >> a.sh1;
+    const uint64_t l0 = q0 & 0xffffffull, l1 = q1 & 0xffffffull;
+    q0 = a.d ? q0 : (l0 | (l0 << 24));
+    q1 = a.d ? q1 : (l1 | (l1 << 24));
+    int t0[6], t1[6];
+#pragma unroll
+    for (int k = 0; k < 6; ++k) { t0[k] = (int)((q0 >> (8 * k)) & 0xff); t1[k] = (int)((q1 >> (8 * k)) & 0xff); }
+    if (area_fast) {
+#pragma unroll
+        for (int c = 0; c < 3; ++c) v[c] = (t0[c] + t0[c + 3] + t1[c] + t1[c + 3] + 2) >> 2;
+        return;
+    }
+    int sx, sy;
+    float fx, fy;
+    resize_linear_x(w, scale_x, x, sx, fx);
+    resize_linear_y(scale_y, y, sy, fy);
+    const int a0 = coef11((1.0f - fx) * 2048.0f), a1 = coef11(fx * 2048.0f);
+    const int b0 = coef11((1.0f - fy) * 2048.0f), b1 = coef11(fy * 2048.0f);
+#pragma unroll
+    for (int c = 0; c < 3; ++c) {
+        const int r0 = t0[c] * a0 + t0[3 + c] * a1;
+        const int r1 = t1[c] * a0 + t1[3 + c] * a1;
+        v[c] = (((b0 * (r0 >> 4)) >> 16) + ((b1 * (r1 >> 4)) >> 16) + 2) >> 2;
+        v[c] = min(255, max(0, v[c]));
+    }
+}
+
+__device__ __forceinline__ void resize_linear_px(const uint8_t *src, long long stride, int h, int w, double scale_x,
+                                                 double scale_y, int area_fast, int x, int y, int v[3])
+{
+    const ResizeAddr a = resize_linear_addr(stride, h, w, scale_x, scale_y, area_fast, x, y);
+    const ResizeTaps t = resize_wide_ok(stride, h, w) ? resize_linear_load<true>(src, a) : resize_linear_load<false>(src, a);
+    resize_linear_finish(stride, h, w, scale_x, scale_y, area_fast, x, y, t, v);
+}
+
+__device__ __forceinline__ bool letterbox_inside(const PreImage &im, int x, int y) { return x < im.new_w && y < im.new_h; }
+
+__device__ __forceinline__ uint2 letterbox_nhwc4(const int v[3])
+{
+    const uint32_t r = __float_as_uint((float)v[2]) >> 16, g = __float_as_uint((float)v[1]) >> 16;
+    const uint32_t bl = __float_as_uint((float)v[0]) >> 16;
+    return make_uint2(r | (g << 16), bl);
+}
+
+}
diff --git a/rs-face-detection_amd/python/rfd_hip/__init__.py b/rs-face-detection_amd/python/rfd_hip/__init__.py
--- a/rs-face-detection_amd/python/rfd_hip/__init__.py
+++ b/rs-face-detection_amd/python/rfd_hip/__init__.py
@@ -110,7 +110,7 @@
     "rfd_detect_batch_device", "rfd_sync", "rfd_set_stream", "rfd_preprocess", "rfd_forward", "rfd_decode_nms",
     "rfd_nms_sorted", "_nms", "rfd_get_stats", "rfd_get_config", "rfd_set_thresholds", "rfd_set_profiling",
     "rfd_get_conv_profile", "rfd_get_op_profile", "rfd_debug_tensor_io", "rfd_debug_run_ops", "rfd_debug_run_chain", "rfd_debug_pass_chains", "rfd_debug_buffer_io",
-    "rfd_debug_set_conv_tile", "rfd_debug_op_kernels", "rfd_debug_op_kernels_static", "rfd_debug_set_concurrency", "rfd_debug_persistent_kernel", "rfd_debug_poke_nms_flag", "rfd_selection_config_default",
+    "rfd_debug_set_conv_tile", "rfd_debug_op_kernels", "rfd_debug_op_kernels_static", "rfd_debug_set_concurrency", "rfd_debug_set_fused_preprocess", "rfd_debug_run_chain_from_frames", "rfd_debug_persistent_kernel", "rfd_debug_poke_nms_flag", "rfd_selection_config_default",
     "rfd_select_faces", "rfd_detect_select_batch", "rfd_save_weights", "rfd_load_weights",
     "rfd_alignment_config_default", "rfd_align_faces", "rfd_detect_select_align_batch",
     "rfd_host_alloc", "rfd_host_free", "rfd_submit_batch", "rfd_collect_batch",
@@ -182,6 +182,8 @@
     L.rfd_debug_op_kernels.argtypes = [vp, ci, ci, ci, C.c_char_p, ci]
     L.rfd_debug_op_kernels_static.argtypes = [ci] * 9 + [C.c_char_p, ci]
     L.rfd_debug_poke_nms_flag.argtypes = [vp, ci]
+    L.rfd_debug_set_fused_preprocess.argtypes = [vp, ci]
+    L.rfd_debug_run_chain_from_frames.argtypes = [vp, C.POINTER(rfd_image), ci, ci, ci]
     L.rfd_debug_persistent_kernel.argtypes = [ci, C.POINTER(C.c_char_p), C.POINTER(C.c_size_t)]
     L.rfd_save_weights.argtypes = [vp, C.c_char_p]
     L.rfd_load_weights.argtypes = [vp, C.c_char_p]
@@ -695,6 +697,15 @@
         _check(self._L.rfd_debug_set_concurrency(self._ctx, int(multi_stream), int(split_min_part), int(split_max_parts),
                                                  int(use_graph)))
 
+    def debug_set_fused_preprocess(self, on=True):
+        _check(self._L.rfd_debug_set_fused_preprocess(self._ctx, 1 if on else 0))
+
+    def debug_run_from_frames(self, frames, last_op, batch_off=0):
+        arr = (rfd_image * len(frames))()
+        for i, (p, h, w, pitch) in enumerate(frames):
+            arr[i].data, arr[i].height, arr[i].width, arr[i].stride = p, h, w, pitch
+        return _check(self._L.rfd_debug_run_chain_from_frames(self._ctx, arr, len(frames), last_op, batch_off)) == 1
+
     def debug_run(self, n, first_op, last_op, batch_off=0, co_running=False):
         if batch_off == 0 and not co_running:
             _check(self._L.rfd_debug_run_ops(self._ctx, n, first_op, last_op))
```

New measurement: 8185 images/s. 0.988x the previous value.
